# tszalay/poreseq

Hardware: AMD Instinct MI355X
Metric: kb consensus refined/sec at 10x coverage (higher is better)
Workload: dtype f64; 1 GPU; poreseq consensus, 10 kb region, 10x synthetic coverage (BASELINE configs[1]), full Mutate.py schedule per region; a step is 280 independent regions per GPU = 14 lock-step batches; the batches of the timed steps run step by step (a step's batches all finish before the next step's start) through 14 batch slots (host threads) per GPU; marshalling + H2D of the events, host greedy steps and D2H inside; region_bases=10000, events=10, regions_per_gpu=280, batches_in_flight=14, step_barrier=True, parallelism=280 regions x 1 GPU(s), 14 host thread(s) per GPU, no data-path collective

## Files before the change

### poreseq_amd/_capi.py

```python
import ctypes as C
import os

import numpy as np

_HERE = os.path.dirname(os.path.abspath(__file__))
HIP_LIB = os.path.join(_HERE, "csrc", "libporeseq_hip.so")

c_dp = C.POINTER(C.c_double)
c_i32p = C.POINTER(C.c_int32)
c_i64p = C.POINTER(C.c_int64)
c_u8p = C.POINTER(C.c_uint8)


class PsParams(C.Structure):
    _fields_ = [("lik_offset", C.c_double), ("scoring_width", C.c_int32),
                ("realign_width", C.c_int32), ("verbose", C.c_int32)]


class PoreseqError(Exception):
    pass


SYMBOLS = {
    "ps_last_error": (C.c_char_p, []),
    "ps_backend_name": (C.c_char_p, []),
    "ps_info": (C.c_int, [C.c_char_p, C.c_int64]),
    "ps_align_create": (C.c_int, [C.POINTER(C.c_void_p), C.c_char_p, C.c_int64, C.c_int32, c_i64p,
                                  c_dp, c_dp, c_dp, c_dp, c_dp, c_dp, C.c_char_p, c_i64p,
                                  C.POINTER(PsParams)]),
    "ps_align_destroy": (None, [C.c_void_p]),
    "ps_align_set_scoring_width": (C.c_int, [C.c_void_p, C.c_int32]),
    "ps_align_new_call": (C.c_int, [C.c_void_p, C.c_int32]),
    "ps_align_n_events": (C.c_int32, [C.c_void_p]),
    "ps_align_n_levels": (C.c_int64, [C.c_void_p, C.c_int32]),
    "ps_align_sequence_length": (C.c_int64, [C.c_void_p]),
    "ps_align_get_sequence": (C.c_int, [C.c_void_p, C.c_char_p, C.c_int64]),
    "ps_align_get_event_refs": (C.c_int, [C.c_void_p, C.c_int32, c_dp, c_dp]),
    "ps_muts_create": (C.c_int, [C.POINTER(C.c_void_p), C.c_int64, c_i32p, c_i64p, C.c_char_p,
                                 c_i64p, C.c_char_p, c_dp]),
    "ps_muts_destroy": (None, [C.c_void_p]),
    "ps_muts_count": (C.c_int64, [C.c_void_p]),
    "ps_muts_orig_bytes": (C.c_int64, [C.c_void_p]),
    "ps_muts_mut_bytes": (C.c_int64, [C.c_void_p]),
    "ps_muts_export": (C.c_int, [C.c_void_p, c_i32p, c_i64p, C.c_char_p, c_i64p, C.c_char_p, c_dp]),
    "ps_seqs_destroy": (None, [C.c_void_p]),
    "ps_seqs_count": (C.c_int64, [C.c_void_p]),
    "ps_seqs_bytes": (C.c_int64, [C.c_void_p]),
    "ps_seqs_export": (C.c_int, [C.c_void_p, c_i64p, C.c_char_p]),
    "ps_score_alignments": (C.c_int, [C.c_void_p, c_dp, c_dp]),
    "ps_find_point_mutations": (C.c_int, [C.c_void_p, C.POINTER(C.c_void_p)]),
    "ps_find_mutations": (C.c_int, [C.c_void_p, C.c_int32, c_i64p, C.c_char_p, C.POINTER(C.c_void_p)]),
    "ps_score_mutations": (C.c_int, [C.c_void_p, C.c_void_p, C.POINTER(C.c_void_p)]),
    "ps_score_mutation_deltas": (C.c_int, [C.c_void_p, C.c_void_p, c_dp]),
    "ps_make_mutations": (C.c_int, [C.c_void_p, C.c_void_p, c_i32p]),
    "ps_viterbi_mutate": (C.c_int, [C.c_void_p, C.c_int32, C.c_double, C.c_double, C.c_double,
                                    C.c_double, C.c_int32, C.POINTER(C.c_void_p)]),
    "ps_srand": (C.c_int, [C.c_uint32]),
    "ps_rand_draw": (C.c_int, [C.c_int64, c_dp]),
    "ps_rng_create": (C.c_int, [C.POINTER(C.c_void_p), C.c_uint32]),
    "ps_rng_destroy": (None, [C.c_void_p]),
    "ps_seqs_create": (C.c_int, [C.POINTER(C.c_void_p), C.c_int64, c_i64p, C.c_char_p]),
    "ps_batch_score_alignments": (C.c_int, [C.c_int32, C.POINTER(C.c_void_p), C.POINTER(c_dp), C.POINTER(c_dp)]),
    "ps_batch_find_mutations": (C.c_int, [C.c_int32, C.POINTER(C.c_void_p), C.POINTER(C.c_void_p), C.POINTER(C.c_void_p)]),
    "ps_batch_score_mutations": (C.c_int, [C.c_int32, C.POINTER(C.c_void_p), C.POINTER(C.c_void_p), C.POINTER(C.c_void_p)]),
    "ps_batch_make_mutations": (C.c_int, [C.c_int32, C.POINTER(C.c_void_p), C.POINTER(C.c_void_p), c_i32p]),
    "ps_batch_viterbi_mutate": (C.c_int, [C.c_int32, C.POINTER(C.c_void_p), C.POINTER(C.c_void_p), C.c_int32, C.c_double,
                                          C.c_double, C.c_double, C.c_double, C.POINTER(C.c_void_p)]),
    "ps_swfull": (C.c_int, [C.c_char_p, C.c_int64, C.c_char_p, C.c_int64, c_i32p, c_dp, c_i32p,
                            c_i32p, C.c_int64, c_i64p]),
    "ps_seq_to_states": (C.c_int, [C.c_char_p, C.c_int64, c_i32p, c_i64p]),
    "ps_debug_fill": (C.c_int, [C.c_void_p, C.c_int32, C.c_int32, c_dp, c_dp, c_u8p, c_u8p]),
    "ps_set_sweep_min": (C.c_int, [C.c_int32]),
    "ps_set_sweep2_min": (C.c_int, [C.c_int32]),
    "ps_set_sparse_min": (C.c_int, [C.c_int32]),
    "ps_set_sweep_form": (C.c_int, [C.c_int32, C.c_int32]),
    "ps_set_device_fraction": (C.c_int, [C.c_double]),
    "ps_prof_enable": (C.c_int, [C.c_int32]),
    "ps_prof_reset": (C.c_int, []),
    "ps_prof_get": (C.c_int, [C.c_char_p, c_dp, c_i64p, c_dp]),
    "ps_prof_units": (C.c_int, [C.c_char_p, c_dp]),
}


def _dp(a):
    return a.ctypes.data_as(c_dp)


def _f64(a):
    return np.ascontiguousarray(a, dtype=np.float64)


class CApi:

    def __init__(self, path):
        if not os.path.exists(path):
            raise PoreseqError("poreseq_amd: native library not found: %s "
                               "(build it with `python -c 'import __graft_entry__ as g; g.build()'`)" % path)
        self.path = path
        self.lib = C.CDLL(path)
        for name, (res, args) in SYMBOLS.items():
            fn = getattr(self.lib, name)
            fn.restype = res
            fn.argtypes = args

    def check(self, rc):
        if rc != 0:
            msg = self.lib.ps_last_error()
            raise PoreseqError("%s failed (%d): %s" % (os.path.basename(self.path), rc,
                                                      msg.decode() if msg else "?"))

    def backend_name(self):
        return self.lib.ps_backend_name().decode()

    def info(self):
        buf = C.create_string_buffer(1024)
        self.check(self.lib.ps_info(buf, 1024))
        return buf.value.decode()

    def align_create(self, sequence, events, params):
        E = len(events)
        for ev in events:
            ev.makecontiguous()
        lens = [int(ev.mean.size) for ev in events]
        off = np.zeros(E + 1, dtype=np.int64)
        off[1:] = np.cumsum(lens)
        cat = lambda name: (_f64(np.concatenate([_f64(getattr(ev, name)) for ev in events]))
                            if E else np.zeros(0))
        mean, stdv, ra, rl = cat("mean"), cat("stdv"), cat("ref_align"), cat("ref_like")
        for ev, n in zip(events, lens):
            if not (ev.stdv.size == n and ev.ref_align.size == n and ev.ref_like.size == n):
                raise PoreseqError("event arrays differ in length")
        model = np.zeros((E, 4, 1024), dtype=np.float64)
        trans = np.zeros((E, 4), dtype=np.float64)
        for e, ev in enumerate(events):
            m = ev.model
            model[e, 0], model[e, 1] = _f64(m.level_mean), _f64(m.level_stdv)
            model[e, 2], model[e, 3] = _f64(m.sd_mean), _f64(m.sd_stdv)
            trans[e] = (m.prob_skip, m.prob_stay, m.prob_extend, m.prob_insert)
        evseqs = [(getattr(ev, "sequence", "") or "").encode("ascii") for ev in events]
        eoff = np.zeros(E + 1, dtype=np.int64)
        eoff[1:] = np.cumsum([len(s) for s in evseqs])
        epool = b"".join(evseqs)
        pp = PsParams(4.5, 150, 300, 0)
        if "verbose" in params:
            pp.verbose = int(params["verbose"])
        if "lik_offset" in params:
            pp.lik_offset = float(params["lik_offset"])
        if "realign_width" in params:
            pp.realign_width = int(params["realign_width"])
        if "scoring_width" in params:
            pp.scoring_width = int(params["scoring_width"])
        seq = sequence.encode("ascii")
        h = C.c_void_p()
        self.check(self.lib.ps_align_create(C.byref(h), seq, len(seq), E, off.ctypes.data_as(c_i64p),
                                            _dp(mean), _dp(stdv), _dp(ra), _dp(rl), _dp(model),
                                            _dp(trans), epool, eoff.ctypes.data_as(c_i64p), C.byref(pp)))
        return h

    def align_destroy(self, h):
        self.lib.ps_align_destroy(h)

    def align_sequence(self, h):
        n = self.lib.ps_align_sequence_length(h)
        buf = C.create_string_buffer(max(int(n), 1))
        self.check(self.lib.ps_align_get_sequence(h, buf, n))
        return buf.raw[:n].decode("ascii")

    def align_update_events(self, h, events):
        for e, ev in enumerate(events):
            n = int(self.lib.ps_align_n_levels(h, e))
            ra = np.empty(n, dtype=np.float64)
            rl = np.empty(n, dtype=np.float64)
            self.check(self.lib.ps_align_get_event_refs(h, e, _dp(ra), _dp(rl)))
            ev.ref_align[:] = ra
            ev.ref_like[:] = rl

    def muts_create(self, muts, with_scores=False):
        n = len(muts)
        start = np.array([int(m.start) for m in muts], dtype=np.int32)
        origs = [m.orig.encode("ascii") for m in muts]
        mutsb = [m.mut.encode("ascii") for m in muts]
        oo = np.zeros(n + 1, dtype=np.int64)
        oo[1:] = np.cumsum([len(s) for s in origs])
        mo = np.zeros(n + 1, dtype=np.int64)
        mo[1:] = np.cumsum([len(s) for s in mutsb])
        score = np.array([float(m.score) for m in muts], dtype=np.float64) if with_scores else None
        h = C.c_void_p()
        self.check(self.lib.ps_muts_create(C.byref(h), n, start.ctypes.data_as(c_i32p),
                                           oo.ctypes.data_as(c_i64p), b"".join(origs),
                                           mo.ctypes.data_as(c_i64p), b"".join(mutsb),
                                           _dp(score) if score is not None else None))
        return h

    def muts_export(self, h):
        n = int(self.lib.ps_muts_count(h))
        ob, mb = int(self.lib.ps_muts_orig_bytes(h)), int(self.lib.ps_muts_mut_bytes(h))
        start = np.zeros(n, dtype=np.int32)
        oo = np.zeros(n + 1, dtype=np.int64)
        mo = np.zeros(n + 1, dtype=np.int64)
        score = np.zeros(n, dtype=np.float64)
        op = C.create_string_buffer(max(ob, 1))
        mp = C.create_string_buffer(max(mb, 1))
        self.check(self.lib.ps_muts_export(h, start.ctypes.data_as(c_i32p), oo.ctypes.data_as(c_i64p), op,
                                           mo.ctypes.data_as(c_i64p), mp, _dp(score)))
        ops, mps = op.raw[:ob].decode("ascii"), mp.raw[:mb].decode("ascii")
        orig = [ops[oo[i]:oo[i + 1]] for i in range(n)]
        mut = [mps[mo[i]:mo[i + 1]] for i in range(n)]
        return start, orig, mut, score

    def muts_destroy(self, h):
        self.lib.ps_muts_destroy(h)

    def seqs_export(self, h):
        n = int(self.lib.ps_seqs_count(h))
        nb = int(self.lib.ps_seqs_bytes(h))
        off = np.zeros(n + 1, dtype=np.int64)
        pool = C.create_string_buffer(max(nb, 1))
        self.check(self.lib.ps_seqs_export(h, off.ctypes.data_as(c_i64p), pool))
        s = pool.raw[:nb].decode("ascii")
        return [s[off[i]:off[i + 1]] for i in range(n)]

    def score_alignments(self, h, n_events, likes_len=None):
        scores = np.zeros(n_events, dtype=np.float64)
        likes = np.zeros(likes_len, dtype=np.float64) if likes_len is not None else None
        self.check(self.lib.ps_score_alignments(h, _dp(scores), _dp(likes) if likes is not None else None))
        return (scores, likes) if likes is not None else scores

    def find_point_mutations(self, h):
        out = C.c_void_p()
        self.check(self.lib.ps_find_point_mutations(h, C.byref(out)))
        return out

    def find_mutations(self, h, seqs):
        bs = [s.encode("ascii") for s in seqs]
        off = np.zeros(len(bs) + 1, dtype=np.int64)
        off[1:] = np.cumsum([len(b) for b in bs])
        out = C.c_void_p()
        self.check(self.lib.ps_find_mutations(h, len(bs), off.ctypes.data_as(c_i64p), b"".join(bs), C.byref(out)))
        return out

    def score_mutations(self, h, hm):
        out = C.c_void_p()
        self.check(self.lib.ps_score_mutations(h, hm, C.byref(out)))
        return out

    def score_mutation_deltas(self, h, hm, n_events, n_muts):
        out = np.zeros((int(n_events), int(n_muts)), dtype=np.float64)
        if out.size:
            self.check(self.lib.ps_score_mutation_deltas(h, hm, _dp(out)))
        return out

    def make_mutations(self, h, hm):
        nb = C.c_int32(0)
        self.check(self.lib.ps_make_mutations(h, hm, C.byref(nb)))
        return int(nb.value)

    def viterbi_mutate(self, h, nkeep, skip, stay, mmin, mmax, verbose):
        out = C.c_void_p()
        self.check(self.lib.ps_viterbi_mutate(h, nkeep, skip, stay, mmin, mmax, int(bool(verbose)), C.byref(out)))
        try:
            return self.seqs_export(out)
        finally:
            self.lib.ps_seqs_destroy(out)

    @staticmethod
    def _harr(handles):
        arr = (C.c_void_p * len(handles))()
        for i, h in enumerate(handles):
            arr[i] = h.value if isinstance(h, C.c_void_p) else h
        return arr

    def rng_create(self, seed=1):
        h = C.c_void_p()
        self.check(self.lib.ps_rng_create(C.byref(h), int(seed)))
        return h

    def rng_destroy(self, h):
        self.lib.ps_rng_destroy(h)

    def seqs_create(self, seqs):
        bs = [s.encode("ascii") for s in seqs]
        off = np.zeros(len(bs) + 1, dtype=np.int64)
        off[1:] = np.cumsum([len(b) for b in bs])
        h = C.c_void_p()
        self.check(self.lib.ps_seqs_create(C.byref(h), len(bs), off.ctypes.data_as(c_i64p), b"".join(bs)))
        return h

    def seqs_destroy(self, h):
        self.lib.ps_seqs_destroy(h)

    def batch_score_alignments(self, handles, n_events):
        n = len(handles)
        scores = [np.zeros(max(int(e), 1), dtype=np.float64) for e in n_events]
        sp = (c_dp * n)(*[_dp(a) for a in scores])
        self.check(self.lib.ps_batch_score_alignments(n, self._harr(handles), sp, None))
        return [a[:int(e)] for a, e in zip(scores, n_events)]

    def batch_find_mutations(self, handles, seqs_handles):
        n = len(handles)
        out = (C.c_void_p * n)()
        self.check(self.lib.ps_batch_find_mutations(n, self._harr(handles), self._harr(seqs_handles), out))
        return [C.c_void_p(out[i]) for i in range(n)]

    def batch_score_mutations(self, handles, muts_handles):
        n = len(handles)
        out = (C.c_void_p * n)()
        self.check(self.lib.ps_batch_score_mutations(n, self._harr(handles), self._harr(muts_handles), out))
        return [C.c_void_p(out[i]) for i in range(n)]

    def batch_make_mutations(self, handles, muts_handles):
        n = len(handles)
        nb = np.zeros(max(n, 1), dtype=np.int32)
        self.check(self.lib.ps_batch_make_mutations(n, self._harr(handles), self._harr(muts_handles), nb.ctypes.data_as(c_i32p)))
        return [int(x) for x in nb[:n]]

    def batch_viterbi_mutate(self, handles, rngs, nkeep, skip, stay, mmin, mmax):
        n = len(handles)
        out = (C.c_void_p * n)()
        self.check(self.lib.ps_batch_viterbi_mutate(n, self._harr(handles), self._harr(rngs), nkeep, skip, stay, mmin, mmax, out))
        res = []
        for i in range(n):
            h = C.c_void_p(out[i])
            try:
                res.append(self.seqs_export(h))
            finally:
                self.lib.ps_seqs_destroy(h)
        return res

    def srand(self, seed):
        self.check(self.lib.ps_srand(int(seed)))

    def rand_draw(self, n):
        out = np.zeros(int(n), dtype=np.float64)
        self.check(self.lib.ps_rand_draw(int(n), _dp(out)))
        return out

    def swfull(self, s1, s2):
        b1, b2 = s1.encode("ascii"), s2.encode("ascii")
        cap = len(b1) + len(b2) + 1
        i1 = np.zeros(cap, dtype=np.int32)
        i2 = np.zeros(cap, dtype=np.int32)
        score = C.c_int32(0)
        acc = C.c_double(0)
        n = C.c_int64(0)
        self.check(self.lib.ps_swfull(b1, len(b1), b2, len(b2), C.byref(score), C.byref(acc),
                                      i1.ctypes.data_as(c_i32p), i2.ctypes.data_as(c_i32p), cap, C.byref(n)))
        return int(score.value), float(acc.value), i1[:n.value].copy(), i2[:n.value].copy()

    def seq_to_states(self, s):
        b = s.encode("ascii")
        st = np.zeros(max(len(b), 1), dtype=np.int32)
        n = C.c_int64(0)
        self.check(self.lib.ps_seq_to_states(b, len(b), st.ctypes.data_as(c_i32p), C.byref(n)))
        return st[:n.value].copy()

    def debug_fill(self, h, ev, direction, n_levels, n_states):
        shape = (n_levels + 1, n_states + 1)
        main = np.zeros(shape)
        stay = np.zeros(shape)
        sm = np.zeros(shape, dtype=np.uint8)
        ss = np.zeros(shape, dtype=np.uint8)
        self.check(self.lib.ps_debug_fill(h, ev, direction, _dp(main), _dp(stay),
                                          sm.ctypes.data_as(c_u8p), ss.ctypes.data_as(c_u8p)))
        return main, stay, sm, ss

    def set_sweep_min(self, n):
        self.check(self.lib.ps_set_sweep_min(int(n)))

    def set_sweep2_min(self, n):
        self.check(self.lib.ps_set_sweep2_min(int(n)))

    def set_sparse_min(self, n):
        self.check(self.lib.ps_set_sparse_min(int(n)))

    def set_sweep_form(self, rows_per_lane, wavefronts=1):
        self.check(self.lib.ps_set_sweep_form(int(rows_per_lane), int(wavefronts)))

    def set_device_fraction(self, fraction):
        self.check(self.lib.ps_set_device_fraction(float(fraction)))

    def prof_enable(self, on):
        self.check(self.lib.ps_prof_enable(int(on)))

    def prof_reset(self):
        self.check(self.lib.ps_prof_reset())

    def prof_units(self, name):
        u = C.c_double(0)
        self.check(self.lib.ps_prof_units(name.encode(), C.byref(u)))
        return float(u.value)

    def prof_get(self, name):
        ms, n, b = C.c_double(0), C.c_int64(0), C.c_double(0)
        self.check(self.lib.ps_prof_get(name.encode(), C.byref(ms), C.byref(n), C.byref(b)))
        return float(ms.value), int(n.value), float(b.value)


_hip = None


def load_hip():
    global _hip
    if _hip is None:
        _hip = CApi(HIP_LIB)
    return _hip
```

### poreseq_amd/csrc/ps_api.cpp

```cpp
#include <algorithm>
#include <cmath>
#include <cstring>
#include <memory>

#include "ps_host.h"

using namespace ps;

struct ps_align { Align a; };
struct ps_muts { std::vector<Mut> v; };
struct ps_seqs { std::vector<std::string> v; };
struct ps_rng { RandState* s = nullptr; ~ps_rng() { if (s) rand_state_free(s); } };

#define NEED_RT()            \
    Runtime* rt = nullptr;   \
    PS_TRY(runtime(&rt))

extern "C" {

const char* ps_last_error(void) { return last_error(); }
const char* ps_backend_name(void) { return "hip-gfx950"; }
int ps_info(char* out, int64_t cap) {
    if (!out || cap <= 0) return fail(PS_ERR_BAD_ARG, "ps_info");
    const std::string s = info_string();
    const size_t n = std::min<size_t>(s.size(), (size_t)cap - 1);
    memcpy(out, s.data(), n);
    out[n] = 0;
    return PS_OK;
}

int ps_align_create(ps_align** out, const char* seq, int64_t seq_len, int32_t n_events,
                    const int64_t* level_off, const double* mean, const double* stdv,
                    const double* ref_align, const double* ref_like, const double* model,
                    const double* trans, const char* evseq, const int64_t* evseq_off,
                    const ps_params* params) {
    if (!out || !seq || seq_len < 0 || n_events < 0 ||
        (n_events && (!level_off || !mean || !stdv || !ref_align || !ref_like || !model || !trans)))
        return fail(PS_ERR_BAD_ARG, "ps_align_create: bad argument");
    NEED_RT();
    std::unique_ptr<ps_align> h(new ps_align());
    PS_TRY(h->a.create(rt, seq, seq_len, n_events, level_off, mean, stdv, ref_align, ref_like, model, trans,
                       evseq, evseq_off, params));
    *out = h.release();
    return PS_OK;
}
void ps_align_destroy(ps_align* a) { delete a; }
int ps_align_set_scoring_width(ps_align* a, int32_t w) {
    if (!a) return fail(PS_ERR_BAD_ARG, "null handle");
    a->a.par.scoring_width = w;
    return PS_OK;
}
int ps_align_new_call(ps_align* a, int32_t w) {
    if (!a) return fail(PS_ERR_BAD_ARG, "null handle");
    a->a.par.scoring_width = w;
    a->a.seqlikes.clear();
    return PS_OK;
}
int32_t ps_align_n_events(const ps_align* a) { return a ? a->a.E : 0; }
int64_t ps_align_n_levels(const ps_align* a, int32_t e) { return (a && e >= 0 && e < a->a.E) ? a->a.n[e] : -1; }
int64_t ps_align_sequence_length(const ps_align* a) { return a ? (int64_t)a->a.bases.size() : -1; }
int ps_align_get_sequence(const ps_align* a, char* out, int64_t cap) {
    if (!a || !out || cap < (int64_t)a->a.bases.size()) return fail(PS_ERR_BAD_ARG, "ps_align_get_sequence");
    memcpy(out, a->a.bases.data(), a->a.bases.size());
    return PS_OK;
}
int ps_align_get_event_refs(const ps_align* ca, int32_t e, double* ra, double* rl) {
    ps_align* a = const_cast<ps_align*>(ca);
    if (!a || e < 0 || e >= a->a.E) return fail(PS_ERR_BAD_ARG, "ps_align_get_event_refs");
    NEED_RT();
    PS_TRY(a->a.refs_to_host(rt));
    const int64_t o = a->a.off[e];
    if (ra) memcpy(ra, a->a.h_ra.data() + o, a->a.n[e] * sizeof(double));
    if (rl) memcpy(rl, a->a.h_rl.data() + o, a->a.n[e] * sizeof(double));
    return PS_OK;
}

int ps_muts_create(ps_muts** out, int64_t n, const int32_t* start, const int64_t* oo, const char* op,
                   const int64_t* mo, const char* mp, const double* score) {
    if (!out || n < 0 || (n && (!start || !oo || !mo))) return fail(PS_ERR_BAD_ARG, "ps_muts_create");
    ps_muts* m = new ps_muts();
    m->v.resize(n);
    for (int64_t i = 0; i < n; i++) {
        m->v[i].start = start[i];
        if (oo[i + 1] > oo[i]) m->v[i].orig.assign(op + oo[i], op + oo[i + 1]);
        if (mo[i + 1] > mo[i]) m->v[i].mut.assign(mp + mo[i], mp + mo[i + 1]);
        m->v[i].score = score ? score[i] : -1e-6;
    }
    *out = m;
    return PS_OK;
}
void ps_muts_destroy(ps_muts* m) { delete m; }
int64_t ps_muts_count(const ps_muts* m) { return m ? (int64_t)m->v.size() : 0; }
int64_t ps_muts_orig_bytes(const ps_muts* m) { int64_t t = 0; if (m) for (auto& x : m->v) t += x.orig.size(); return t; }
int64_t ps_muts_mut_bytes(const ps_muts* m) { int64_t t = 0; if (m) for (auto& x : m->v) t += x.mut.size(); return t; }
int ps_muts_export(const ps_muts* m, int32_t* start, int64_t* oo, char* op, int64_t* mo, char* mp, double* score) {
    if (!m) return fail(PS_ERR_BAD_ARG, "ps_muts_export");
    int64_t a = 0, b = 0;
    for (size_t i = 0; i < m->v.size(); i++) {
        const Mut& x = m->v[i];
        if (start) start[i] = x.start;
        if (oo) oo[i] = a;
        if (mo) mo[i] = b;
        if (op) memcpy(op + a, x.orig.data(), x.orig.size());
        if (mp) memcpy(mp + b, x.mut.data(), x.mut.size());
        a += x.orig.size(); b += x.mut.size();
        if (score) score[i] = x.score;
    }
    if (oo) oo[m->v.size()] = a;
    if (mo) mo[m->v.size()] = b;
    return PS_OK;
}

void ps_seqs_destroy(ps_seqs* s) { delete s; }
int64_t ps_seqs_count(const ps_seqs* s) { return s ? (int64_t)s->v.size() : 0; }
int64_t ps_seqs_bytes(const ps_seqs* s) { int64_t t = 0; if (s) for (auto& x : s->v) t += x.size(); return t; }
int ps_seqs_export(const ps_seqs* s, int64_t* off, char* pool) {
    if (!s) return fail(PS_ERR_BAD_ARG, "ps_seqs_export");
    int64_t a = 0;
    for (size_t i = 0; i < s->v.size(); i++) {
        if (off) off[i] = a;
        if (pool) memcpy(pool + a, s->v[i].data(), s->v[i].size());
        a += s->v[i].size();
    }
    if (off) off[s->v.size()] = a;
    return PS_OK;
}

int ps_score_alignments(ps_align* a, double* scores, double* likes) {
    if (!a || (!scores && a->a.E)) return fail(PS_ERR_BAD_ARG, "ps_score_alignments");
    NEED_RT();
    return score_alignments(rt, &a->a, scores, likes);
}
int ps_find_point_mutations(ps_align* a, ps_muts** out) {
    if (!a || !out) return fail(PS_ERR_BAD_ARG, "ps_find_point_mutations");
    ps_muts* m = new ps_muts();
    find_point_mutations(&a->a, &m->v);
    *out = m;
    return PS_OK;
}
int ps_find_mutations(ps_align* a, int32_t n, const int64_t* off, const char* pool, ps_muts** out) {
    if (!a || !out || n < 0 || (n && (!off || !pool))) return fail(PS_ERR_BAD_ARG, "ps_find_mutations");
    NEED_RT();
    std::vector<std::string> seeds;
    for (int i = 0; i < n; i++) seeds.emplace_back(pool + off[i], pool + off[i + 1]);
    std::unique_ptr<ps_muts> m(new ps_muts());
    PS_TRY(find_mutations(rt, &a->a, seeds, &m->v));
    *out = m.release();
    return PS_OK;
}
int ps_score_mutations(ps_align* a, const ps_muts* in, ps_muts** out) {
    if (!a || !in || !out) return fail(PS_ERR_BAD_ARG, "ps_score_mutations");
    NEED_RT();
    std::unique_ptr<ps_muts> m(new ps_muts());
    PS_TRY(score_mutations(rt, &a->a, in->v, &m->v));
    *out = m.release();
    return PS_OK;
}
int ps_score_mutation_deltas(ps_align* a, const ps_muts* in, double* deltas) {
    if (!a || !in || !deltas) return fail(PS_ERR_BAD_ARG, "ps_score_mutation_deltas");
    NEED_RT();
    std::vector<Mut> scored;
    std::vector<double*> dout(1, deltas);
    return score_mutations_multi(rt, {&a->a}, {&in->v}, {&scored}, &dout);
}
int ps_make_mutations(ps_align* a, const ps_muts* in, int32_t* nb) {
    if (!a || !in || !nb) return fail(PS_ERR_BAD_ARG, "ps_make_mutations");
    NEED_RT();
    int n = 0;
    PS_TRY(make_mutations(rt, &a->a, in->v, &n));
    *nb = n;
    return PS_OK;
}
int ps_viterbi_mutate(ps_align* a, int32_t nkeep, double skip, double stay, double mmin, double mmax,
                      int32_t verbose, ps_seqs** out) {
    if (!a || !out || a->a.E == 0 || nkeep < 0) return fail(PS_ERR_BAD_ARG, "ps_viterbi_mutate");
    NEED_RT();
    std::unique_ptr<ps_seqs> s(new ps_seqs());
    PS_TRY(viterbi_mutate(rt, &a->a, nkeep, skip, stay, mmin, mmax, &s->v, verbose != 0));
    *out = s.release();
    return PS_OK;
}
int ps_rng_create(ps_rng** out, uint32_t seed) {
    if (!out) return fail(PS_ERR_BAD_ARG, "ps_rng_create");
    ps_rng* r = new ps_rng();
    r->s = rand_state_new(seed);
    *out = r;
    return PS_OK;
}
void ps_rng_destroy(ps_rng* r) { delete r; }
int ps_seqs_create(ps_seqs** out, int64_t n, const int64_t* off, const char* pool) {
    if (!out || n < 0 || (n && (!off || !pool))) return fail(PS_ERR_BAD_ARG, "ps_seqs_create");
    ps_seqs* s = new ps_seqs();
    for (int64_t i = 0; i < n; i++) s->v.emplace_back(pool + off[i], pool + off[i + 1]);
    *out = s;
    return PS_OK;
}
static int batch_handles(int32_t n, ps_align* const* a, std::vector<Align*>* as) {
    if (n < 0 || (n && !a)) return fail(PS_ERR_BAD_ARG, "batch: bad handle array");
    for (int i = 0; i < n; i++) {
        if (!a[i]) return fail(PS_ERR_BAD_ARG, "batch: null handle");
        for (int j = 0; j < i; j++) if (a[j] == a[i]) return fail(PS_ERR_BAD_ARG, "batch: the same handle twice");
        as->push_back(&a[i]->a);
    }
    return PS_OK;
}
int ps_batch_score_alignments(int32_t n, ps_align* const* a, double* const* scores, double* const* likes) {
    std::vector<Align*> as;
    PS_TRY(batch_handles(n, a, &as));
    if (n && !scores) return fail(PS_ERR_BAD_ARG, "ps_batch_score_alignments");
    NEED_RT();
    std::vector<double*> sc(n), lk(n);
    for (int i = 0; i < n; i++) {
        if (!scores[i] && as[i]->E) return fail(PS_ERR_BAD_ARG, "ps_batch_score_alignments: null scores");
        sc[i] = scores[i]; lk[i] = likes ? likes[i] : nullptr;
    }
    return score_alignments_multi(rt, as, sc, lk);
}
int ps_batch_find_mutations(int32_t n, ps_align* const* a, const ps_seqs* const* seeds, ps_muts** out) {
    std::vector<Align*> as;
    PS_TRY(batch_handles(n, a, &as));
    if (n && (!seeds || !out)) return fail(PS_ERR_BAD_ARG, "ps_batch_find_mutations");
    NEED_RT();
    std::vector<std::unique_ptr<ps_muts>> m(n);
    std::vector<const std::vector<std::string>*> sd(n);
    std::vector<std::vector<Mut>*> o(n);
    for (int i = 0; i < n; i++) {
        if (!seeds[i]) return fail(PS_ERR_BAD_ARG, "ps_batch_find_mutations: null seeds");
        m[i].reset(new ps_muts()); sd[i] = &seeds[i]->v; o[i] = &m[i]->v;
    }
    PS_TRY(find_mutations_multi(rt, as, sd, o));
    for (int i = 0; i < n; i++) out[i] = m[i].release();
    return PS_OK;
}
int ps_batch_score_mutations(int32_t n, ps_align* const* a, const ps_muts* const* muts, ps_muts** out) {
    std::vector<Align*> as;
    PS_TRY(batch_handles(n, a, &as));
    if (n && (!muts || !out)) return fail(PS_ERR_BAD_ARG, "ps_batch_score_mutations");
    NEED_RT();
    std::vector<std::unique_ptr<ps_muts>> m(n);
    std::vector<const std::vector<Mut>*> in(n);
    std::vector<std::vector<Mut>*> o(n);
    for (int i = 0; i < n; i++) {
        if (!muts[i]) return fail(PS_ERR_BAD_ARG, "ps_batch_score_mutations: null list");
        m[i].reset(new ps_muts()); in[i] = &muts[i]->v; o[i] = &m[i]->v;
    }
    PS_TRY(score_mutations_multi(rt, as, in, o));
    for (int i = 0; i < n; i++) out[i] = m[i].release();
    return PS_OK;
}
int ps_batch_make_mutations(int32_t n, ps_align* const* a, const ps_muts* const* scored, int32_t* n_bases) {
    std::vector<Align*> as;
    PS_TRY(batch_handles(n, a, &as));
    if (n && (!scored || !n_bases)) return fail(PS_ERR_BAD_ARG, "ps_batch_make_mutations");
    NEED_RT();
    std::vector<std::vector<Mut>> in(n);
    for (int i = 0; i < n; i++) if (!scored[i]) return fail(PS_ERR_BAD_ARG, "ps_batch_make_mutations: null list");
    par_for(n, [&](int i) { in[i] = scored[i]->v; });
    std::vector<int> nb;
    PS_TRY(make_mutations_multi(rt, as, std::move(in), &nb));
    for (int i = 0; i < n; i++) n_bases[i] = nb[i];
    return PS_OK;
}
int ps_batch_viterbi_mutate(int32_t n, ps_align* const* a, ps_rng* const* rng, int32_t nkeep, double skip, double stay,
                            double mmin, double mmax, ps_seqs** out) {
    std::vector<Align*> as;
    PS_TRY(batch_handles(n, a, &as));
    if (n && !out) return fail(PS_ERR_BAD_ARG, "ps_batch_viterbi_mutate");
    if (nkeep < 0) return fail(PS_ERR_BAD_ARG, "ps_batch_viterbi_mutate: nkeep");
    for (Align* x : as) if (x->E == 0) return fail(PS_ERR_BAD_ARG, "ps_batch_viterbi_mutate: no events");
    NEED_RT();
    std::vector<std::unique_ptr<ps_seqs>> s(n);
    std::vector<RandState*> rs(n, nullptr);
    std::vector<std::vector<std::string>*> o(n);
    for (int i = 0; i < n; i++) { s[i].reset(new ps_seqs()); o[i] = &s[i]->v; rs[i] = (rng && rng[i]) ? rng[i]->s : nullptr; }
    PS_TRY(viterbi_mutate_multi(rt, as, rs, nkeep, skip, stay, mmin, mmax, o));
    for (int i = 0; i < n; i++) out[i] = s[i].release();
    return PS_OK;
}

int ps_swfull(const char* s1, int64_t n1, const char* s2, int64_t n2, int32_t* score, double* acc,
              int32_t* i1, int32_t* i2, int64_t cap, int64_t* np) {
    if (!s1 || !s2 || n1 < 0 || n2 < 0 || !np) return fail(PS_ERR_BAD_ARG, "ps_swfull");
    NEED_RT();
    int sc = 0; double ac = 0;
    std::vector<int> a, b;
    PS_TRY(sw_device(rt, std::string(s1, n1), std::string(s2, n2), &sc, &ac, &a, &b));
    if ((int64_t)a.size() > cap) return fail(PS_ERR_BAD_ARG, "ps_swfull: index capacity too small");
    if (score) *score = sc;
    if (acc) *acc = ac;
    for (size_t k = 0; k < a.size(); k++) { if (i1) i1[k] = a[k]; if (i2) i2[k] = b[k]; }
    *np = (int64_t)a.size();
    return PS_OK;
}
int ps_seq_to_states(const char* seq, int64_t n, int32_t* st, int64_t* ns) {
    if (!seq || n < 0 || !ns) return fail(PS_ERR_BAD_ARG, "ps_seq_to_states");
    std::vector<int> v = states_of(std::string(seq, n));
    if (st) std::copy(v.begin(), v.end(), st);
    *ns = (int64_t)v.size();
    return PS_OK;
}

int ps_debug_fill(ps_align* a, int32_t e, int32_t dir, double* main, double* stay, uint8_t* sm, uint8_t* ss) {
    if (!a || e < 0 || e >= a->a.E || !main || dir < 0 || dir > 1) return fail(PS_ERR_BAD_ARG, "ps_debug_fill");
    NEED_RT();
    return debug_fill(rt, &a->a, e, dir, main, stay, sm, ss);
}

int ps_srand(uint32_t seed) { rand_seed(seed); return PS_OK; }
int ps_rand_draw(int64_t n, double* out) {
    if (n < 0 || (n && !out)) return fail(PS_ERR_BAD_ARG, "ps_rand_draw");
    for (int64_t k = 0; k < n; k++) out[k] = rand_next() / (double(RAND_MAX) + 1);
    return PS_OK;
}

int ps_set_sweep_min(int32_t n) { sweep_min_set(n); return PS_OK; }
int ps_set_sweep2_min(int32_t n) { sweep2_min_set(n); return PS_OK; }
int ps_set_sparse_min(int32_t n) { sparse_min_set(n); return PS_OK; }
int ps_set_device_fraction(double f) {
    if (f > 1.0) return fail(PS_ERR_BAD_ARG, "ps_set_device_fraction: a fraction in (0, 1]; <= 0 restores the default");
    device_fraction_set(f);
    return PS_OK;
}
int ps_set_sweep_form(int32_t K, int32_t NW) {
    if (K <= 0 && NW > 0 && NW != 1 && NW != 2 && NW != 4) return fail(PS_ERR_BAD_ARG, "ps_set_sweep_form: 1, 2 or 4 wavefronts per sweep");
    if (K > 0 && !sweep_form_exists(K, NW)) return fail(PS_ERR_BAD_ARG, "ps_set_sweep_form: no such form (rows per lane, wavefronts)");
    sweep_form_set(K, NW);
    return PS_OK;
}

int ps_prof_enable(int32_t on) {
    NEED_RT();
    prof_flush(rt);
    rt->prof_on = on != 0;
    rt->prof_defer = on == 2;
    return PS_OK;
}
int ps_prof_reset(void) {
    NEED_RT();
    prof_flush(rt);
    rt->prof.clear();
    return PS_OK;
}
int ps_prof_get(const char* name, double* ms, int64_t* n, double* bytes) {
    NEED_RT();
    prof_flush(rt);
    Prof p;
    if (name) { auto it = rt->prof.find(name); if (it != rt->prof.end()) p = it->second; }
    if (ms) *ms = p.ms;
    if (n) *n = p.launches;
    if (bytes) *bytes = p.bytes;
    return PS_OK;
}

int ps_prof_units(const char* name, double* units) {
    NEED_RT();
    prof_flush(rt);
    Prof p;
    if (name) { auto it = rt->prof.find(name); if (it != rt->prof.end()) p = it->second; }
    if (units) *units = p.units;
    return PS_OK;
}

}
```

### poreseq_amd/csrc/ps_find.cpp

```cpp
#include <algorithm>
#include <cmath>
#include <cstdlib>
#include <cstring>
#include <map>
#include <thread>

#include "ps_host.h"
#include "ps_sw.h"

namespace ps {

static double max_batch_bytes() { return device_share_bytes(); }

static void fillinds(SwResult& al) {
    if (al.a.empty()) return;
    int i1 = al.a[0], i2 = al.b[0];
    for (size_t k = 0; k < al.a.size(); k++) {
        if (al.a[k] > 0) i1 = al.a[k]; else al.a[k] = i1;
        if (al.b[k] > 0) i2 = al.b[k]; else al.b[k] = i2;
    }
}

static int argmax(const std::vector<double>& v) { return (int)(std::max_element(v.begin(), v.end()) - v.begin()); }

static int extract_edits(Align* a, const std::vector<std::string>& seeds, std::vector<SwResult>& als, const std::vector<double>& base,
                         std::vector<Mut>* out) {
    const size_t L = a->bases.size();
    const int S = (int)seeds.size();
    std::vector<std::vector<double>> dl(S);
    for (int k = 0; k < S; k++) {
        SwResult& al = als[k];
        const std::vector<double>& rl = a->seqlikes[seeds[k]];
        for (size_t q = 0; q < al.a.size(); q++) { al.a[q] -= 2; al.b[q] -= 2; }
        while (!al.a.empty() && (al.a[0] < 0 || al.b[0] < 0)) { al.a.erase(al.a.begin()); al.b.erase(al.b.begin()); }
        const size_t n = al.a.size();
        std::vector<double> x(n), y(n);
        for (size_t q = 0; q < n; q++) {
            x[q] = (size_t)al.a[q] < base.size() ? base[al.a[q]] : 0.0;
            y[q] = (size_t)al.b[q] < rl.size() ? rl[al.b[q]] : 0.0;
        }
        for (size_t q = n; q-- > 1;) { x[q] -= x[q - 1]; y[q] -= y[q - 1]; }
        if (n) { x[0] = 0; y[0] = 0; }
        std::vector<double>& cs = dl[k];
        cs.resize(n);
        double run = 0;
        for (size_t q = 0; q < n; q++) {
            run += y[q] - x[q];
            if (run < 0) run = 0;
            cs[q] = run;
            if (std::fabs(x[q] - y[q]) < 1e-5) cs[q] = 0;
        }
    }
    const size_t BLK = 128;
    std::vector<std::vector<double>> bmax(S);
    auto block_refresh = [&](int k, size_t blk) {
        const std::vector<double>& v = dl[k];
        const size_t lo = blk * BLK, hi = std::min(v.size(), lo + BLK);
        double m = v[lo];
        for (size_t q = lo + 1; q < hi; q++) if (v[q] > m) m = v[q];
        bmax[k][blk] = m;
    };
    auto seed_argmax = [&](int k) -> int {
        const std::vector<double>& bm = bmax[k];
        size_t bb = 0;
        for (size_t q = 1; q < bm.size(); q++) if (bm[q] > bm[bb]) bb = q;
        const std::vector<double>& v = dl[k];
        const size_t lo = bb * BLK, hi = std::min(v.size(), lo + BLK);
        size_t at = lo;
        for (size_t q = lo + 1; q < hi; q++) if (v[q] > v[at]) at = q;
        return (int)at;
    };
    std::vector<double> top(S, 0.0);
    std::vector<int> topi(S, 0);
    for (int k = 0; k < S; k++) {
        if (dl[k].empty()) continue;
        bmax[k].resize((dl[k].size() + BLK - 1) / BLK);
        for (size_t blk = 0; blk < bmax[k].size(); blk++) block_refresh(k, blk);
        topi[k] = seed_argmax(k);
        top[k] = dl[k][topi[k]];
    }
    while (out->size() < L / 3) {
        const int w = argmax(top);
        std::vector<double>& v = dl[w];
        if (v.empty()) break;
        const int ind = topi[w];
        if (v[ind] < 0.25) break;
        int i1 = (int)(std::find(v.begin() + ind, v.end(), 0.0) - v.begin());
        int i0 = -1;
        for (int q = ind; q >= 0; q--) if (v[q] == 0) { i0 = q; break; }
        if (i0 < 0) i0 = 0;
        if (i1 < 0) i1 = 0;
        if ((size_t)i0 >= v.size()) i0 = (int)v.size() - 1;
        if ((size_t)i1 >= v.size()) i1 = (int)v.size() - 1;
        const int s1 = als[w].a[i0], s2 = als[w].b[i0], e1 = als[w].a[ind], e2 = als[w].b[ind];
        Mut m;
        m.start = s1;
        if ((size_t)s1 > a->bases.size() || (size_t)s2 > seeds[w].size()) return PS_ERR_BAD_ARG;
        m.orig = a->bases.substr(s1, (size_t)(e1 - s1));
        m.mut = seeds[w].substr(s2, (size_t)(e2 - s2));
        while (!m.orig.empty() && !m.mut.empty() && m.orig.front() == m.mut.front()) {
            m.orig.erase(m.orig.begin()); m.mut.erase(m.mut.begin()); m.start++;
        }
        while (!m.orig.empty() && !m.mut.empty() && m.orig.back() == m.mut.back()) { m.orig.pop_back(); m.mut.pop_back(); }
        if (!m.orig.empty() || !m.mut.empty()) out->push_back(m);
        std::fill(v.begin() + i0, v.begin() + i1 + 1, 0.0);
        for (size_t blk = (size_t)i0 / BLK; blk <= (size_t)i1 / BLK; blk++) block_refresh(w, blk);
        topi[w] = seed_argmax(w);
        top[w] = v[topi[w]];
    }
    return PS_OK;
}

int find_mutations_multi(Runtime* rt, const std::vector<Align*>& as, const std::vector<const std::vector<std::string>*>& seeds,
                         const std::vector<std::vector<Mut>*>& outs) {
    Tick tk("find_mutations");
    const int R = (int)as.size();
    for (int r = 0; r < R; r++) outs[r]->clear();
    std::vector<std::pair<const std::string*, const std::string*>> pairs;
    std::vector<int> pair0(R + 1, 0);
    for (int r = 0; r < R; r++) {
        pair0[r] = (int)pairs.size();
        for (const std::string& s : *seeds[r]) pairs.push_back({&as[r]->bases, &s});
    }
    pair0[R] = (int)pairs.size();
    auto sw_bytes = [&](size_t k) {
        const double n1 = (double)pairs[k].first->size(), n2 = (double)pairs[k].second->size();
        return 4.0 * ((n1 / 64 + 1) * (n2 + 8) + (n2 / 64 + 1) * (n1 + 1)) + 8.0 * (n1 + n2 + 2);
    };
    double sw_cap = device_share_bytes() / 8;
    auto sw_chunk_end = [&](size_t k0) {
        double acc = 0;
        size_t k = k0;
        for (; k < pairs.size(); k++) { const double add = sw_bytes(k); if (k > k0 && acc + add > sw_cap) break; acc += add; }
        return k;
    };
    typedef std::vector<std::pair<const std::string*, const std::string*>> SwIn;
    SwJob swjob;
    size_t sw_first = sw_chunk_end(0);
    {
        const int rc = sw_launch(rt, SwIn(pairs.begin(), pairs.begin() + sw_first), &swjob);
        if (rc == PS_ERR_NOMEM && sw_first > 1) { sw_first = 0; swjob = SwJob(); }
        else PS_TRY(rc);
    }
    tk.lap("sw enqueue");
    std::vector<std::vector<double>> base(R), sc(R);
    std::vector<double*> scp(R), lkp(R);
    for (int r = 0; r < R; r++) {
        base[r].assign(std::max<size_t>(as[r]->bases.size(), 4) + 1, 0.0);
        sc[r].assign(std::max(as[r]->E, 1), 0.0);
        scp[r] = sc[r].data(); lkp[r] = base[r].data();
    }
    const int rc_base = score_alignments_multi(rt, as, scp, lkp);
    tk.lap("base realign");
    std::vector<SwResult> als_all;
    PS_TRY(sw_finish(rt, &swjob, &als_all));
    PS_TRY(rc_base);
    for (size_t k0 = sw_first; k0 < pairs.size();) {
        const size_t k1 = sw_chunk_end(k0);
        std::vector<SwResult> part;
        const int rc = sw_batch(rt, SwIn(pairs.begin() + k0, pairs.begin() + k1), &part);
        if (rc == PS_ERR_NOMEM && k1 - k0 > 1) { sw_cap *= 0.5; continue; }
        PS_TRY(rc);
        for (SwResult& r : part) als_all.push_back(std::move(r));
        k0 = k1;
    }
    if (sw_first < pairs.size()) { static const bool trace = getenv("PORESEQ_TRACE") != nullptr; if (trace) fprintf(stderr, "[ps] smith-waterman: %zu pairs, %zu with the realign, the rest in chunks\n", pairs.size(), sw_first); }
    if (pairs.empty()) return PS_OK;
    if (R == 1 && as[0]->par.verbose) {
        fputs("Finding mutations", stderr);
        for (size_t k = 0; k < seeds[0]->size(); k++) fputc('.', stderr);
        fputc('\n', stderr);
        fflush(stderr);
    }
    par_for((int)als_all.size(), [&](int k) { fillinds(als_all[k]); });
    tk.lap("smith-waterman");
    struct Need { int r, k; std::vector<int> states; };
    std::vector<Need> need;
    for (int r = 0; r < R; r++) {
        Align* a = as[r];
        const std::vector<std::string>& sd = *seeds[r];
        std::map<std::string, int> seen;
        for (int k = 0; k < (int)sd.size(); k++) {
            if (!a->seqlikes[sd[k]].empty()) continue;
            if (seen.count(sd[k])) continue;
            seen[sd[k]] = k;
            if (a->E) need.push_back({r, k, {}});
            else a->seqlikes[sd[k]] = std::vector<double>(sd[k].size(), 0.0);
        }
    }
    if (!need.empty()) {
        {
            for (int r = 0; r < R; r++) PS_TRY(as[r]->refs_to_host_async(rt));
            PS_HIP(hipStreamSynchronize(rt->stream));
            for (int r = 0; r < R; r++) as[r]->refs_finish();
        }
        par_for((int)need.size(), [&](int q) { need[q].states = states_of((*seeds[need[q].r])[need[q].k]); });
        const double cap = max_batch_bytes();
        size_t q0 = 0;
        int p_seen = 0;
        size_t limit = (size_t)-1;
        while (q0 < need.size()) {
            size_t q1 = q0;
            double bytes = 0;
            size_t nref = 0;
            while (q1 < need.size()) {
                const Align* a = as[need[q1].r];
                const int P = std::max(p_seen, guess_slots(a));
                double add = 0;
                for (int e = 0; e < a->E; e++)
                    add += sweep_enabled() && sweep_guess_k(a->par.realign_width) ? fwd_job_bytes(a, a->n[e], (int)need[q1].states.size())
                                                                                  : ((double)a->n[e] + need[q1].states.size() + 1 + MAT_FRONT + MAT_BACK) * P * 18.0;
                if (q1 > q0 && (bytes + add > cap || q1 - q0 >= limit)) break;
                bytes += add; nref += (size_t)a->ntot; q1++;
            }
            const size_t stage_mark = rt->stage.mark();
            double* h_ra = (double*)rt->stage.alloc(std::max<size_t>(nref, 1) * sizeof(double));
            if (!h_ra) return fail(PS_ERR_NOMEM, "hipHostMalloc (staging arena)");
            std::vector<size_t> roff(q1 - q0 + 1, 0);
            for (size_t q = q0; q < q1; q++) roff[q - q0 + 1] = roff[q - q0] + (size_t)as[need[q].r]->ntot;
            par_for((int)(q1 - q0), [&](int qq) {
                const Need& nd = need[q0 + qq];
                const Align* a = as[nd.r];
                const SwResult& al = als_all[pair0[nd.r] + nd.k];
                double* dst = h_ra + roff[qq];
                for (int64_t t = 0; t < a->ntot; t++) {
                    const int ra = (int)a->h_ra[t];
                    double v = 0.0;
                    if (!al.a.empty() && !(ra < al.a.front() || ra > al.a.back())) {
                        const size_t k = std::lower_bound(al.a.begin(), al.a.end(), ra) - al.a.begin();
                        v = k < al.b.size() ? (double)al.b[k] : 0.0;
                    }
                    dst[t] = v;
                }
            });
            tk.lap("remap (host)");
            DBuf& rb = rt->buf("seed_refs");
            PS_TRY(rb.ensure((size_t)3 * std::max<size_t>(nref, 1) * sizeof(double)));
            double* d_ra = rb.as<double>();
            double* d_rl = d_ra + nref;
            double* d_ri = d_rl + nref;
            if (nref) PS_HIP(hipMemcpyAsync(d_ra, h_ra, nref * sizeof(double), hipMemcpyHostToDevice, rt->stream));
            PS_HIP(hipMemsetAsync(d_rl, 0, std::max<size_t>(nref, 1) * sizeof(double), rt->stream));
            size_t njobs = 0;
            for (size_t q = q0; q < q1; q++) njobs += as[need[q].r]->E;
            DBuf& ob = rt->buf("seed_out");
            PS_TRY(ob.ensure(njobs * sizeof(JobOut)));
            PS_HIP(hipMemsetAsync(ob.p, 0, njobs * sizeof(JobOut), rt->stream));
            std::vector<JobSpec> specs;
            for (size_t q = q0; q < q1; q++) {
                Align* a = as[need[q].r];
                for (int e = 0; e < a->E; e++) {
                    JobSpec s;
                    s.a = a; s.ev = e; s.states = &need[q].states;
                    const size_t o = roff[q - q0] + a->off[e];
                    s.ra = d_ra + o; s.rl = d_rl + o; s.ri = d_ri + o;
                    s.out = ob.as<JobOut>() + specs.size();
                    specs.push_back(s);
                }
            }
            Batch b;
            PS_TRY(b.build(rt, specs, 1, 0));
            PS_TRY(launch_updaterefs(rt, b.d));
            tk.lap("seed batch build");
            {
                const int rc = realign(rt, b, q1 - q0 > 1 ? 1.2 * cap : 0.0);
                if (rc == PS_SPLIT) {
                    { static const bool trace = getenv("PORESEQ_TRACE") != nullptr; if (trace) fprintf(stderr, "[ps] seed chunk of %zu cut again: %d slots per anti-diagonal, %d guessed\n", q1 - q0, b.P, std::max(p_seen, 0)); }
                    p_seen = std::max(p_seen, b.P);
                    limit = std::max<size_t>(1, (q1 - q0) / 2);
                    PS_HIP(hipStreamSynchronize(rt->stream));
                    rt->stage.release(stage_mark);
                    continue;
                }
                PS_TRY(rc);
            }
            p_seen = std::max(p_seen, b.P);
            std::vector<std::vector<double>> lks(q1 - q0);
            bool on_device = true;
            for (size_t q = q0; q < q1; q++) if ((int)need[q].states.size() > likes_max_states()) on_device = false;
            if (on_device) {
                std::vector<LikeGroup> groups(q1 - q0);
                int64_t out_tot = 0;
                int job = 0;
                for (size_t q = q0; q < q1; q++) {
                    LikeGroup& g = groups[q - q0];
                    const std::string& sd = (*seeds[need[q].r])[need[q].k];
                    g.job0 = job; g.njobs = as[need[q].r]->E; job += g.njobs;
                    g.C = (int)need[q].states.size(); g.len = (int)sd.size();
                    g.out_off = out_tot; out_tot += g.len;
                }
                DBuf& gb = rt->buf("like_groups");
                DBuf& lb = rt->buf("like_out");
                PS_TRY(gb.ensure(groups.size() * sizeof(LikeGroup)));
                PS_TRY(lb.ensure((size_t)std::max<int64_t>(out_tot, 1) * sizeof(double)));
                PS_TRY(rt->up(gb.p, groups.data(), groups.size() * sizeof(LikeGroup)));
                PS_TRY(launch_likes(rt, b.d, gb.as<LikeGroup>(), (int)groups.size(), lb.as<double>()));
                double* h_lk = nullptr;
                PS_TRY(rt->down(&h_lk, lb.p, (size_t)out_tot));
                PS_HIP(hipStreamSynchronize(rt->stream));
                tk.lap("seed realign + D2H");
                for (size_t q = q0; q < q1; q++) lks[q - q0].assign(h_lk + groups[q - q0].out_off, h_lk + groups[q - q0].out_off + groups[q - q0].len);
            } else {
            double *r_ra = nullptr, *r_rl = nullptr;
            PS_TRY(rt->down(&r_ra, d_ra, nref));
            PS_TRY(rt->down(&r_rl, d_rl, nref));
            PS_HIP(hipStreamSynchronize(rt->stream));
            tk.lap("seed realign + D2H");
            par_for((int)(q1 - q0), [&](int qq) {
                const Need& nd = need[q0 + qq];
                const Align* a = as[nd.r];
                const std::string& sd = (*seeds[nd.r])[nd.k];
                std::vector<double>& lk = lks[qq];
                lk.assign(std::max<size_t>(sd.size(), 4) + 1, 0.0);
                for (int e = 0; e < a->E; e++) {
                    const size_t o = roff[qq] + a->off[e];
                    accumulate_likes(r_ra + o, r_rl + o, a->n[e], (int)nd.states.size(), lk.data());
                }
                lk.resize(sd.size());
            });
            }
            for (size_t q = q0; q < q1; q++) as[need[q].r]->seqlikes[(*seeds[need[q].r])[need[q].k]] = std::move(lks[q - q0]);
            rt->stage.release(stage_mark);
            q0 = q1;
        }
    }
    tk.lap("seed likes");
    std::vector<int> rcs(R, PS_OK);
    par_for(R, [&](int r) {
        std::vector<SwResult> als(als_all.begin() + pair0[r], als_all.begin() + pair0[r + 1]);
        rcs[r] = extract_edits(as[r], *seeds[r], als, base[r], outs[r]);
    });
    for (int r = 0; r < R; r++) if (rcs[r] != PS_OK) return fail(rcs[r], "FindMutations: alignment index outside the sequence");
    tk.lap("extract");
    return PS_OK;
}

int find_mutations(Runtime* rt, Align* a, const std::vector<std::string>& seeds, std::vector<Mut>* out) {
    return find_mutations_multi(rt, {a}, {&seeds}, {out});
}

inline int succ(int st, int k, int j) { return ((st << (2 * j)) & (NS - 1)) + k; }
inline char base_at(int st, int k) { return "ACGT"[3 & (st >> (2 * (4 - k)))]; }

static std::string path_to_bases(const std::vector<int>& st) {
    std::string s;
    int cur = st[0];
    s.push_back(base_at(cur, 0));
    for (size_t i = 1; i < st.size(); i++) {
        if (cur == st[i]) continue;
        bool hit = false;
        for (int n = 1; n <= 4 && !hit; n++)
            for (int k = 0; k < (1 << (2 * n)); k++)
                if (succ(cur, k, n) == st[i]) {
                    for (int b = 1; b <= n; b++) s.push_back(base_at(cur, b));
                    cur = st[i]; hit = true; break;
                }
        if (!hit) { cur = st[i]; s.push_back(base_at(cur, 0)); }
    }
    for (int b = 1; b <= 4; b++) s.push_back(base_at(cur, b));
    return s;
}

struct RandState {
    random_data rd;
    char st[128];
    bool init = false;
};
namespace { thread_local RandState t_rand; }
static void rs_seed(RandState* r, unsigned seed) {
    memset(&r->rd, 0, sizeof(r->rd));
    initstate_r(seed, r->st, sizeof(r->st), &r->rd);
    r->init = true;
}
static int rs_next(RandState* r) {
    if (!r->init) rs_seed(r, 1);
    int32_t v = 0;
    random_r(&r->rd, &v);
    return (int)v;
}
void rand_seed(unsigned seed) { rs_seed(&t_rand, seed); }
int rand_next() { return rs_next(&t_rand); }
RandState* rand_state_new(unsigned seed) { RandState* r = new RandState(); rs_seed(r, seed); return r; }
void rand_state_free(RandState* r) { delete r; }
void rand_state_seed(RandState* r, unsigned seed) { rs_seed(r, seed); }
int rand_state_next(RandState* r) { return rs_next(r ? r : &t_rand); }

namespace {
struct VitGather { std::vector<double> obsin; int T = 0; };
}

static void vit_gather(const Align* a, const double* h_ri, const JobOut* info, VitGather* g) {
    const int E = a->E;
    int maxpos = 0;
    for (int e = 0; e < E; e++) {
        if (!info[e].has_index) continue;
        const double* ri = h_ri + a->off[e];
        for (int t = 0; t < a->n[e]; t++) {
            const double v = ri[t];
            if (v >= 0.0 && v < 1e9 && v == std::floor(v)) maxpos = std::max(maxpos, (int)v);
        }
    }
    std::vector<std::vector<int>> first(E);
    for (int e = 0; e < E; e++) {
        if (!info[e].has_index) continue;
        first[e].assign((size_t)maxpos + 1, -1);
        const double* ri = h_ri + a->off[e];
        for (int t = 0; t < a->n[e]; t++) {
            const double v = ri[t];
            if (v >= 0.0 && v <= (double)maxpos && v == std::floor(v)) {
                int& slot = first[e][(size_t)v];
                if (slot < 0) slot = t;
            }
        }
    }
    auto rstart = [&](int e) { return info[e].has_index ? info[e].refstart : -1; };
    auto rend = [&](int e) { return info[e].has_index ? info[e].refend : -1; };
    int refind = rstart(0);
    for (int e = 0; e < E; e++) refind = std::min(refind, rstart(e));
    std::vector<double>& obsin = g->obsin;
    int T = 0;
    while (true) {
        int nl = 0, nal = 0;
        const size_t at = obsin.size();
        obsin.resize(at + (size_t)E * 4, 0.0);
        for (int e = 0; e < E; e++) {
            if (refind < 0 || refind > maxpos || first[e].empty() || first[e][refind] < 0) continue;
            const double* ra = a->h_ra.data() + a->off[e];
            const double* mean = a->h_mean.data() + a->off[e];
            const double* stdv = a->h_stdv.data() + a->off[e];
            int t = first[e][refind], cnt = 1;
            double lsum = 0, ssum = 0;
            lsum += mean[t]; ssum += stdv[t];
            for (t++; t < a->n[e] && ra[t] <= refind; t++)
                if (ra[t] > 0) { lsum += mean[t]; ssum += stdv[t]; cnt++; }
            const double lvl = lsum / cnt, sd = ssum / cnt;
            nl++;
            double* o = obsin.data() + at + (size_t)e * 4;
            o[0] = lvl; o[1] = sd; o[2] = std::log(sd); o[3] = 1.0;
        }
        for (int e = 0; e < E; e++) if (refind >= rstart(e) && refind <= rend(e)) nal++;
        if (nl <= nal * 0.2) {
            obsin.resize(at);
            if (nal == 0) break;
            refind++;
            continue;
        }
        T++;
        refind++;
    }
    g->T = T;
}

static void vit_draw(void* rng, double* rnd, size_t n) {
    RandState* r = (RandState*)rng;
    for (size_t k = 0; k < n; k++) rnd[k] = rand_state_next(r) / (double(RAND_MAX) + 1);
}

int viterbi_mutate_multi(Runtime* rt, const std::vector<Align*>& as, const std::vector<RandState*>& rngs, int nkeep, double skip, double stay,
                         double mmin, double mmax, const std::vector<std::vector<std::string>*>& outs) {
    Tick tk("viterbi_mutate");
    const int R = (int)as.size();
    for (int r = 0; r < R; r++) outs[r]->clear();
    std::vector<double*> h_ri(R, nullptr);
    std::vector<JobOut*> info(R, nullptr);
    for (int r = 0; r < R; r++) {
        PS_TRY(as[r]->refs_to_host_async(rt));
        as[r]->last_stream = (void*)rt->stream;
        PS_TRY(rt->down(&h_ri[r], as[r]->d_ri, (size_t)as[r]->ntot));
        PS_TRY(rt->down(&info[r], as[r]->d_out, (size_t)as[r]->E));
    }
    PS_HIP(hipStreamSynchronize(rt->stream));
    for (int r = 0; r < R; r++) as[r]->refs_finish();
    tk.lap("refs D2H");
    std::vector<VitGather> gath(R);
    par_for(R, [&](int r) { vit_gather(as[r], h_ri[r], info[r], &gath[r]); });
    tk.lap("gather levels");
    std::vector<VitRegionH> regs(R);
    for (int r = 0; r < R; r++) {
        regs[r].E = as[r]->E; regs[r].T = gath[r].T; regs[r].obsin = gath[r].obsin.data(); regs[r].d_model = as[r]->d_model;
        as[r]->last_stream = (void*)rt->stream;
        regs[r].rng = rngs[r]; regs[r].draw = vit_draw;
    }
    std::vector<std::vector<std::vector<int>>> paths;
    {
        auto need = [&](size_t k) { return 26.0 * 1024.0 * (double)regs[k].T + 32.0 * (double)regs[k].T * regs[k].E; };
        double cap = std::max(1e9, 0.9 * device_share_bytes());
        for (size_t k0 = 0; k0 < regs.size();) {
            size_t k1 = k0;
            double acc = 0;
            for (; k1 < regs.size(); k1++) { const double add = need(k1); if (k1 > k0 && acc + add > cap) break; acc += add; }
            std::vector<std::vector<std::vector<int>>> part;
            const int rc = viterbi_device_multi(rt, std::vector<VitRegionH>(regs.begin() + k0, regs.begin() + k1), nkeep, skip, stay, mmin, mmax, &part);
            if (rc == PS_ERR_NOMEM && k1 - k0 > 1) { cap *= 0.5; continue; }
            PS_TRY(rc);
            for (auto& pr : part) paths.push_back(std::move(pr));
            k0 = k1;
        }
    }
    tk.lap("device");
    par_for(R, [&](int r) { for (auto& p : paths[r]) outs[r]->push_back(path_to_bases(p)); });
    tk.lap("paths to bases");
    return PS_OK;
}

int viterbi_mutate(Runtime* rt, Align* a, int nkeep, double skip, double stay, double mmin, double mmax,
                   std::vector<std::string>* out, bool verbose) {
    const int rc = viterbi_mutate_multi(rt, {a}, {nullptr}, nkeep, skip, stay, mmin, mmax, {out});
    if (verbose && rc == PS_OK) {
        fputs("Viterbi", stderr);
        for (size_t k = 200; k <= a->bases.size(); k += 200) fputc('.', stderr);
        fputc('\n', stderr);
        fflush(stderr);
    }
    return rc;
}

}
```

### poreseq_amd/csrc/ps_internal.h

```cpp
#ifndef PS_INTERNAL_H_
#define PS_INTERNAL_H_

#include <hip/hip_runtime.h>
#include <stdint.h>

#include <map>
#include <string>
#include <vector>

#include "../../include/poreseq_hip.h"

namespace ps {

constexpr int NS = PS_N_STATES;
constexpr double BIG = 1e300;

int fail(int code, const std::string& msg);
#define PS_HIP(expr)                                                                          \
    do {                                                                                      \
        hipError_t _e = (expr);                                                               \
        if (_e != hipSuccess)                                                                 \
            return ps::fail(PS_ERR_HIP, std::string(#expr) + ": " + hipGetErrorString(_e));   \
    } while (0)
#define PS_TRY(expr)            \
    do {                        \
        int _rc = (expr);       \
        if (_rc != PS_OK) return _rc; \
    } while (0)

struct DBuf {
    void* p = nullptr;
    size_t cap = 0;
    int ensure(size_t bytes);
    template <class T> T* as() const { return (T*)p; }
};

struct HBuf {
    void* p = nullptr;
    size_t cap = 0;
    int ensure(size_t bytes);
    template <class T> T* as() const { return (T*)p; }
};

struct Stage {
    struct Chunk { char* p; size_t cap; };
    std::vector<Chunk> chunks;
    size_t used = 0;
    bool dirty = false;
    void* alloc(size_t bytes);
    int reset();
    size_t mark() const { return chunks.size() <= 1 ? used : (size_t)-1; }
    void release(size_t m) { if (m != (size_t)-1 && chunks.size() <= 1) used = m; }
};

struct Prof { double ms = 0; int64_t launches = 0; double bytes = 0; double units = 0; };

struct Runtime {
    bool ready = false;
    int device = 0;
    hipStream_t stream = nullptr;
    hipStream_t stream2 = nullptr;
    hipEvent_t ev0 = nullptr, ev1 = nullptr, sw0 = nullptr, sw1 = nullptr;
    std::map<std::string, DBuf> pool;
    std::map<std::string, HBuf> hpool;
    HBuf& hbuf(const std::string& name) { return hpool[name]; }
    std::map<std::string, Prof> prof;
    bool prof_on = false;
    bool prof_defer = false;
    struct ProfPend { hipEvent_t a, b; const char* name; double bytes; };
    std::vector<ProfPend> prof_pend;
    std::vector<hipEvent_t> prof_spare;
    DBuf& buf(const std::string& name) { return pool[name]; }
    Stage stage;
    int up(void* dst, const void* src, size_t bytes, hipStream_t st = nullptr);
    int down(void** hptr, const void* src, size_t bytes, hipStream_t st = nullptr);
    template <class T> int down(T** hptr, const void* src, size_t count) { return down((void**)hptr, src, count * sizeof(T)); }
};
int runtime(Runtime** out);
int second_stream(Runtime* rt, hipStream_t* out);
int live_runtimes();

struct Mut {
    int start = 0;
    std::string orig, mut;
    double score = -1e-6;
};

struct JobOut;
struct JobD {
    const double* model8;
    const double* lev[2];
    const int* st;
    double lsk, lst, lex, lin;
    double lik_offset;
    int n0;
    int C;
    int W;
    int force_inert;
    int P;
    int lbn;
    int K;
    int pitch;
    int NL;
    const int* keep[2];
    int64_t lb_off;
    int64_t lbn_off;
    int64_t mat_off[2];
    int64_t lo_off[2];
    int64_t col_off[2];
    int64_t S;
    double* ra;
    double* rl;
    double* ri;
    JobOut* out;
};

struct JobOut {
    double best;
    int bi, bj;
    int has_index;
    int refstart, refend;
    int inert;
    int term_i, term_w;
};

constexpr int MODEL_ROW_BYTES = 80;
constexpr int MAT_FRONT = 8;
constexpr int MAT_BACK = 16;
constexpr int LO_PAD = 160;

struct SweepJob;
struct BatchD {
    const JobD* jobs;
    int njobs;
    int* lb;
    int* lo;
    int* hi;
    double2* rec;
    unsigned short* flg;
    double* cmax;
    double* pm;
    int* maxw;
    int fastdiv;
    double log2pi;
    const SweepJob* s_sj;
    const int2* s_band;
    const int* s_qlo;
    const int* s_qhi;
};

struct StripBest;
struct SweepJob {
    int64_t codes_off;
    int64_t band_off;
    int64_t q_off;
    int64_t sb_off;
    int T;
    int Q;
};
struct SweepD {
    const SweepJob* sj;
    int2* band;
    int* qlo;
    int* qhi;
    unsigned char* codes;
    StripBest* sb;
    int* maxwin;
    int K;
    int nl;
    int ndir;
    int sparse;
};

struct LikeGroup {
    int job0, njobs;
    int C, len;
    int64_t out_off;
};

int launch_updaterefs(Runtime* rt, const BatchD& b);
int launch_lb(Runtime* rt, const BatchD& b, int which , int maxlbn);
int launch_lo(Runtime* rt, const BatchD& b, int ndir, int64_t maxS);
int launch_fill(Runtime* rt, const BatchD& b, const std::vector<JobD>& jobs, int ndir, int64_t maxS, int P, int64_t ncols);
int launch_backtrace(Runtime* rt, const BatchD& b, int maxn);
int launch_prefix(Runtime* rt, const BatchD& b, int ndir);

struct ScoreArgs {
    int job0, njobs;
    int nitems_per_job;
    int ncolmax;
    int ws;
    const int* m_start;
    const int* m_mlen;
    const int* m_cm;
    const int* m_ncol;
    const int* m_skip;
    const int* m_states;
    const int* m_oldidx;
    const int* r0;
    int nr0;
    double* old;
    double* oldall;
    int64_t oldall_pitch, maxS;
    double* delta;
    double* score;
    const int* cls_items[5];
    int cls_count[5];
};
constexpr int SCORE_CLASSES = 5;
int launch_score(Runtime* rt, const BatchD& b, const ScoreArgs* d_sas, const std::vector<ScoreArgs>& h_sas);
int launch_begin(Runtime* rt, const BatchD& b);
int launch_gather_best(Runtime* rt, const BatchD& b, double* out);

int sw_device(Runtime* rt, const std::string& s1, const std::string& s2, int* score, double* accuracy,
              std::vector<int>* inds1, std::vector<int>* inds2);

struct VitRegionH {
    int E = 0, T = 0;
    const double* obsin = nullptr;
    const double* d_model = nullptr;
    void* rng = nullptr;
    void (*draw)(void* rng, double* out , size_t n) = nullptr;
};
int viterbi_device_multi(Runtime* rt, const std::vector<VitRegionH>& regions, int nkeep, double skip, double stay, double mmin, double mmax,
                         std::vector<std::vector<std::vector<int>>>* paths);

void prof_flush(Runtime* rt);
void prof_begin(Runtime* rt);
void prof_end(Runtime* rt, const char* name, double alg_bytes);

}

#endif
```

### poreseq_amd/csrc/ps_sw.h

```cpp
#ifndef PS_SW_H_
#define PS_SW_H_
#include "ps_internal.h"

namespace ps {

struct SwPair {
    int n1, n2;
    int nrb;
    int ngw;
    int pitch;
    int pad;
    int64_t s1_off, s2_off;
    int64_t row_off;
    int64_t col_off;
    int64_t blk_off;
    int64_t out_off;
    int64_t res_off;
};

struct SwResult { int score = 0; double accuracy = 0; std::vector<int> a, b; };

struct SwJob {
    std::vector<SwPair> pairs;
    std::string pool;
    int* res = nullptr;
    int* outbuf = nullptr;
    int64_t out_tot = 0;
    double cells = 0;
    int np = 0;
    hipStream_t stream = nullptr;
};

typedef std::vector<std::pair<const std::string*, const std::string*>> SwInput;
int sw_launch(Runtime* rt, const SwInput& in, SwJob* job);
int sw_finish(Runtime* rt, SwJob* job, std::vector<SwResult>* out);
int sw_batch(Runtime* rt, const SwInput& in, std::vector<SwResult>* out);

}
#endif
```

### poreseq_amd/csrc/ps_sw.hip

```cpp
#include <cstring>

#include "ps_sw.h"

namespace ps {

constexpr int SWB = 8;
constexpr int SWW = 8;
constexpr int SWW1 = 16;

__device__ __forceinline__ int wave_scan_max(int v) {
    asm("s_nop 1\n\tv_max_i32_dpp %0, %0, %0 row_shr:1 row_mask:0xf bank_mask:0xf\n\t"
        "s_nop 1\n\tv_max_i32_dpp %0, %0, %0 row_shr:2 row_mask:0xf bank_mask:0xf\n\t"
        "s_nop 1\n\tv_max_i32_dpp %0, %0, %0 row_shr:4 row_mask:0xf bank_mask:0xf\n\t"
        "s_nop 1\n\tv_max_i32_dpp %0, %0, %0 row_shr:8 row_mask:0xf bank_mask:0xf\n\t"
        "s_nop 1\n\tv_max_i32_dpp %0, %0, %0 row_bcast:15 row_mask:0xa bank_mask:0xf\n\t"
        "s_nop 1\n\tv_max_i32_dpp %0, %0, %0 row_bcast:31 row_mask:0xc bank_mask:0xf"
        : "+v"(v));
    return v;
}

template <int K, int MODE>
__device__ __forceinline__ unsigned sw_row(int (&G)[K], const int (&c2)[K], const int c1, const int bl, const int bprev,
                                           const int lane, const int lane0, const int target, const int i, const int jfirst, int& fc, int& fr) {
    const int d0 = __builtin_amdgcn_update_dpp(bprev + 8 * (K - 1), G[K - 1], 0x138 , 0xf, 0xf, false);
    int y[K];
    int sd0 = 0, up0 = 0;
#pragma unroll
    for (int k = 0; k < K; k++) {
        const int pen = min(c2[k] ^ c1, 9);
        const int sd = (k ? G[k - 1] + 13 : d0 + (5 - 8 * (K - 1))) - pen;
        const int up = G[k] - 8;
        if (k == 0) { sd0 = sd; up0 = up; }
        y[k] = max(max(sd, up), 8 * k);
    }
    constexpr int NG = (K + 3) / 4;
    int tg[NG];
#pragma unroll
    for (int g = 0; g < NG; g++) {
#pragma unroll
        for (int k = 4 * g + 1; k < min(4 * g + 4, K); k++) y[k] = max(y[k], y[k - 1]);
        const int last = y[min(4 * g + 3, K - 1)];
        tg[g] = g ? max(last, tg[g - 1]) : last;
    }
    int z = tg[NG - 1] + (8 * K * lane - 8 * (K - 1));
    z = max(z, (bl - 8 * K) + lane0);
    z = wave_scan_max(z);
    const int hl8 = __builtin_amdgcn_update_dpp(bl - 8 * K, z, 0x138, 0xf, 0xf, false) + (8 * K - 8 * K * lane - 8);
    unsigned code = 0;
#pragma unroll
    for (int k = 0; k < K; k++) {
        const int gn = k >= 4 ? max(max(y[k], tg[k / 4 - 1]), hl8) : max(y[k], hl8);
        if (MODE == 2 && k == 0) {
            const int l0 = max(hl8, 0), m = max(l0, up0);
            const unsigned step = sd0 >= m ? 3u : (up0 > l0 ? 2u : (hl8 > 0 ? 1u : 0u));
            code = step | (gn > 0 ? 4u : 0u) | (c2[0] == c1 ? 8u : 0u);
        }
        if (MODE == 1) {
            const int col = jfirst + k + 1;
            if (gn == target + 8 * k && col < fc) { fc = col; fr = i; }
        }
        G[k] = gn;
    }
    return code;
}

constexpr int SW_SPIN_LIMIT = 1 << 22;
template <int K, int WW>
__global__ __launch_bounds__(64 * WW) void k_sw_fill(const SwPair* pairs, const char* chars, int* rowsave, int* colsave,
                                                  int* blkmax, int* prog, int* ticket, int* res) {
    __shared__ int s_ticket;
    if (threadIdx.x == 0) s_ticket = atomicAdd(&ticket[blockIdx.y], 1);
    __syncthreads();
    const int ss = s_ticket;
    const SwPair p = pairs[blockIdx.y];
    if (p.n1 <= 0 || p.n2 <= 0 || ss * WW * 64 * K >= p.n2) return;
    int* prog_my = prog + (int64_t)blockIdx.y * gridDim.x + ss;
    const bool has_next = (ss + 1) * WW * 64 * K < p.n2;
    int seen = 0;
    const int t = threadIdx.x, w = t >> 6, l = t & 63;
    const int gw = ss * WW + w;
    const int wfirst = gw * 64 * K;
    const bool wave_on = wfirst < p.n2;
    const int jbase = wfirst + l * K;
    const char* s1 = chars + p.s1_off;
    const char* s2 = chars + p.s2_off;
    int c2[K], G[K], bmk[K];
#pragma unroll
    for (int k = 0; k < K; k++) { c2[k] = jbase + k < p.n2 ? (int)(unsigned char)s2[jbase + k] << 4 : 0; G[k] = 8 * k; bmk[k] = 0; }
    const int lane0 = l ? -(1 << 29) : 0;
    __shared__ int hand[WW][2][SWB];
    const bool keeps = ((jbase + K) & 63) == 0 && jbase + K <= p.n2;
    int* csave = colsave + p.col_off + (int64_t)((jbase + K) >> 6) * (p.n1 + 1);
    const int* cprev = colsave + p.col_off + (int64_t)(wfirst >> 6) * (p.n1 + 1);
    if (wave_on && keeps) csave[0] = 0;
    int bprev = 0, dummy_c = 0, dummy_r = 0;
    const int nchunks = (p.n1 + SWB - 1) / SWB;
    auto fetch = [&](int c, int& ch, int& bd) {
        ch = 1; bd = 0;
        const int i0 = c * SWB;
        if (w == 0 && ss > 0 && c >= 0 && c < nchunks) {
            const int need = min(p.n1, (i0 + SWB + 63) & ~63);
            int spins = 0;
            for (; seen < need && spins < SW_SPIN_LIMIT; spins++) {
                seen = __hip_atomic_load(prog_my - 1, __ATOMIC_ACQUIRE, __HIP_MEMORY_SCOPE_AGENT);
                if (seen < need) __builtin_amdgcn_s_sleep(8);
            }
            if (seen < need && l == 0) atomicOr(&res[p.res_off + 5], 1);
        }
        if (wave_on && c >= 0 && c < nchunks && l < SWB && i0 + l < p.n1) {
            ch = (int)(unsigned char)s1[i0 + l] << 4;
            if (w == 0 && gw > 0) bd = cprev[i0 + 1 + l];
        }
    };
    int ch_nx, bd_nx;
    fetch(0 - w, ch_nx, bd_nx);
    for (int s = 0; s < nchunks + WW - 1; s++) {
        const int c = s - w;
        const int ch1 = ch_nx, bd1 = bd_nx;
        fetch(c + 1, ch_nx, bd_nx);
        if (wave_on && c >= 0 && c < nchunks) {
            const int i0 = c * SWB;
            int bnd = bd1;
            if (w > 0 && l < SWB && i0 + l < p.n1) bnd = hand[w - 1][(s - 1) & 1][l];
            int hl[SWB];
#pragma unroll
            for (int r = 0; r < SWB; r++) hl[r] = 0;
#pragma unroll
            for (int r = 0; r < SWB; r++) {
                if (i0 + r < p.n1) {
                    const int bl = __builtin_amdgcn_readlane(bnd, r), c1 = __builtin_amdgcn_readlane(ch1, r);
                    sw_row<K, 0>(G, c2, c1, bl, bprev, l, lane0, 0, 0, 0, dummy_c, dummy_r);
                    bprev = bl;
#pragma unroll
                    for (int k = 0; k < K; k++) bmk[k] = max(bmk[k], G[k]);
                    const int hlast = G[K - 1] - 8 * (K - 1);
                    if (l == 63) hand[w][s & 1][r] = hlast;
                    hl[r] = hlast;
                }
            }
            if (keeps) {
                if (i0 + SWB <= p.n1) {
                    typedef int v4i_a4 __attribute__((ext_vector_type(4), aligned(4)));
                    *(v4i_a4*)(csave + i0 + 1) = (v4i_a4){hl[0], hl[1], hl[2], hl[3]};
                    *(v4i_a4*)(csave + i0 + 5) = (v4i_a4){hl[4], hl[5], hl[6], hl[7]};
                } else {
#pragma unroll
                    for (int r = 0; r < SWB; r++) if (i0 + r < p.n1) csave[i0 + r + 1] = hl[r];
                }
            }
            const int iend = min(i0 + SWB, p.n1);
            if ((iend & 63) == 0 || iend == p.n1) {
                const int q = (iend - 1) >> 6;
                int bm = 0;
#pragma unroll
                for (int k = 0; k < K; k++) { bm = max(bm, bmk[k] - 8 * k); bmk[k] = 0; }
                for (int o = 32; o; o >>= 1) bm = max(bm, __shfl_xor(bm, o));
                if (l == 0) blkmax[p.blk_off + (int64_t)q * p.ngw + gw] = bm;
                if (has_next && w == WW - 1 && l == 63) __hip_atomic_store(prog_my, iend, __ATOMIC_RELEASE, __HIP_MEMORY_SCOPE_AGENT);
                if (iend < p.n1) {
                    int* rs = rowsave + p.row_off + (int64_t)(q + 1) * p.pitch + jbase;
#pragma unroll
                    for (int k = 0; k < K; k++) if (jbase + k < p.n2) rs[k] = G[k] - 8 * k;
                }
            }
        }
        asm volatile("s_waitcnt lgkmcnt(0)\n\ts_barrier" ::: "memory");
    }
}

typedef unsigned short us2 __attribute__((ext_vector_type(2)));
__device__ __forceinline__ us2 pk_of(unsigned v) { return __builtin_bit_cast(us2, v); }
__device__ __forceinline__ unsigned un_pk(us2 v) { return __builtin_bit_cast(unsigned, v); }
constexpr int PKK = 8;
constexpr int SW_PK_MAXLEN = 13000;

__device__ __forceinline__ void sw_row_pk(unsigned (&P)[4], const unsigned (&sp)[4], const int bl, const int bprev, const int lane8k, const int lane0) {
    const int plast = (int)(P[3] >> 16);
    const int d0 = __builtin_amdgcn_update_dpp(bprev + 8 * PKK, plast, 0x138 , 0xf, 0xf, false) - 8 * PKK;
    us2 y[4];
#pragma unroll
    for (int m = 0; m < 4; m++) {
        const unsigned S = m ? __builtin_amdgcn_alignbit(P[m], P[m - 1], 16) : ((P[0] << 16) | (unsigned)d0);
        const us2 sd = pk_of(S) + pk_of(sp[m]);
        const us2 up = __builtin_elementwise_sub_sat(pk_of(P[m]), (us2){8, 8});
        const us2 fl = {(unsigned short)(8 * (2 * m + 1)), (unsigned short)(8 * (2 * m + 2))};
        y[m] = __builtin_elementwise_max(__builtin_elementwise_max(sd, up), fl);
    }
#pragma unroll
    for (int m = 0; m < 4; m++) {
        const us2 lo = {y[m].x, y[m].x};
        y[m] = __builtin_elementwise_max(y[m], lo);
        if (m) { const us2 ph = {y[m - 1].y, y[m - 1].y}; y[m] = __builtin_elementwise_max(y[m], ph); }
    }
    int z = (int)y[3].y + lane8k;
    z = max(z, bl + lane0);
    z = wave_scan_max(z);
    const int hl = __builtin_amdgcn_update_dpp(bl, z, 0x138, 0xf, 0xf, false) - lane8k;
    const us2 hl2 = {(unsigned short)hl, (unsigned short)hl};
#pragma unroll
    for (int m = 0; m < 4; m++) P[m] = un_pk(__builtin_elementwise_max(y[m], hl2));
}

template <int WW>
__global__ __launch_bounds__(64 * WW) __attribute__((amdgpu_waves_per_eu(8, 8))) void k_sw_fill_pk(const SwPair* pairs, const char* chars, int* rowsave, int* colsave,
                                                       int* blkmax, int* prog, int* ticket, int* res) {
    constexpr int K = PKK;
    __shared__ int s_ticket;
    if (threadIdx.x == 0) s_ticket = atomicAdd(&ticket[blockIdx.y], 1);
    __syncthreads();
    const int ss = s_ticket;
    const SwPair p = pairs[blockIdx.y];
    if (p.n1 <= 0 || p.n2 <= 0 || ss * WW * 64 * K >= p.n2) return;
    int* prog_my = prog + (int64_t)blockIdx.y * gridDim.x + ss;
    const bool has_next = (ss + 1) * WW * 64 * K < p.n2;
    int seen = 0;
    const int t = threadIdx.x, w = t >> 6, l = t & 63;
    const int gw = ss * WW + w;
    const int wfirst = gw * 64 * K;
    const bool wave_on = wfirst < p.n2;
    const int jbase = wfirst + l * K;
    const char* s1 = chars + p.s1_off;
    const char* s2 = chars + p.s2_off;
    __shared__ uint4 s_sp[4][64 * WW];
    unsigned P[4], bmk[4], c2p[4];
    {
        unsigned tb[4][4];
#pragma unroll
        for (int m = 0; m < 4; m++) {
            const unsigned a = jbase + 2 * m < p.n2 ? (unsigned)(unsigned char)s2[jbase + 2 * m] : 0u, b = jbase + 2 * m + 1 < p.n2 ? (unsigned)(unsigned char)s2[jbase + 2 * m + 1] : 0u;
            c2p[m] = (a << 4) | (b << 20);
            auto tab = [&](unsigned ch) { return (a == ch ? 13u : 4u) | ((b == ch ? 13u : 4u) << 16); };
            tb[0][m] = tab('A'); tb[1][m] = tab('C'); tb[2][m] = tab('G'); tb[3][m] = tab('T');
            P[m] = (unsigned)(8 * (2 * m + 1)) | ((unsigned)(8 * (2 * m + 2)) << 16);
            bmk[m] = 0u;
        }
#pragma unroll
        for (int q = 0; q < 4; q++) s_sp[q][threadIdx.x] = make_uint4(tb[q][0], tb[q][1], tb[q][2], tb[q][3]);
    }
    const int lane0 = l ? -(1 << 29) : 0, lane8k = 8 * K * l;
    __shared__ int hand[WW][2][SWB];
    const bool keeps = ((jbase + K) & 63) == 0 && jbase + K <= p.n2;
    int* csave = colsave + p.col_off + (int64_t)((jbase + K) >> 6) * (p.n1 + 1);
    const int* cprev = colsave + p.col_off + (int64_t)(wfirst >> 6) * (p.n1 + 1);
    if (wave_on && keeps) csave[0] = 0;
    int bprev = 0;
    const int nchunks = (p.n1 + SWB - 1) / SWB;
    auto fetch = [&](int c, int& ch, int& bd) {
        ch = 1; bd = 0;
        const int i0 = c * SWB;
        if (w == 0 && ss > 0 && c >= 0 && c < nchunks) {
            const int need = min(p.n1, (i0 + SWB + 63) & ~63);
            int spins = 0;
            for (; seen < need && spins < SW_SPIN_LIMIT; spins++) {
                seen = __hip_atomic_load(prog_my - 1, __ATOMIC_ACQUIRE, __HIP_MEMORY_SCOPE_AGENT);
                if (seen < need) __builtin_amdgcn_s_sleep(8);
            }
            if (seen < need && l == 0) atomicOr(&res[p.res_off + 5], 1);
        }
        if (wave_on && c >= 0 && c < nchunks && l < SWB && i0 + l < p.n1) {
            ch = (int)(unsigned char)s1[i0 + l];
            if (w == 0 && gw > 0) bd = cprev[i0 + 1 + l];
        }
    };
    int ch_nx, bd_nx;
    fetch(0 - w, ch_nx, bd_nx);
    for (int s = 0; s < nchunks + WW - 1; s++) {
        const int c = s - w;
        const int ch1 = ch_nx, bd1 = bd_nx;
        fetch(c + 1, ch_nx, bd_nx);
        if (wave_on && c >= 0 && c < nchunks) {
            const int i0 = c * SWB;
            int bnd = bd1;
            if (w > 0 && l < SWB && i0 + l < p.n1) bnd = hand[w - 1][(s - 1) & 1][l];
            int hl[SWB];
#pragma unroll
            for (int r = 0; r < SWB; r++) hl[r] = 0;
#pragma unroll
            for (int r = 0; r < SWB; r++) {
                if (i0 + r < p.n1) {
                    const int bl = __builtin_amdgcn_readlane(bnd, r), c1 = __builtin_amdgcn_readlane(ch1, r);
                    const int bidx = c1 == 'A' ? 0 : c1 == 'C' ? 1 : c1 == 'G' ? 2 : c1 == 'T' ? 3 : -1;
                    unsigned sp[4];
                    if (bidx >= 0) {
                        const uint4 v = s_sp[bidx][threadIdx.x];
                        sp[0] = v.x; sp[1] = v.y; sp[2] = v.z; sp[3] = v.w;
                    } else {
                        const unsigned c1p = ((unsigned)c1 << 4) | ((unsigned)c1 << 20);
#pragma unroll
                        for (int m = 0; m < 4; m++) sp[m] = un_pk((us2){13, 13} - __builtin_elementwise_min(pk_of(c2p[m] ^ c1p), (us2){9, 9}));
                    }
                    sw_row_pk(P, sp, bl, bprev, lane8k, lane0);
                    bprev = bl;
#pragma unroll
                    for (int m = 0; m < 4; m++) bmk[m] = un_pk(__builtin_elementwise_max(pk_of(bmk[m]), pk_of(P[m])));
                    const int hlast = (int)(P[3] >> 16) - 8 * K;
                    if (l == 63) hand[w][s & 1][r] = hlast;
                    hl[r] = hlast;
                }
            }
            if (keeps) {
                if (i0 + SWB <= p.n1) {
                    typedef int v4i_a4 __attribute__((ext_vector_type(4), aligned(4)));
                    *(v4i_a4*)(csave + i0 + 1) = (v4i_a4){hl[0], hl[1], hl[2], hl[3]};
                    *(v4i_a4*)(csave + i0 + 5) = (v4i_a4){hl[4], hl[5], hl[6], hl[7]};
                } else {
#pragma unroll
                    for (int r = 0; r < SWB; r++) if (i0 + r < p.n1) csave[i0 + r + 1] = hl[r];
                }
            }
            const int iend = min(i0 + SWB, p.n1);
            if ((iend & 63) == 0 || iend == p.n1) {
                const int q = (iend - 1) >> 6;
                int bm = 0;
#pragma unroll
                for (int m = 0; m < 4; m++) {
                    bm = max(bm, (int)(bmk[m] & 0xffffu) - 8 * (2 * m + 1));
                    bm = max(bm, (int)(bmk[m] >> 16) - 8 * (2 * m + 2));
                    bmk[m] = 0u;
                }
                for (int o = 32; o; o >>= 1) bm = max(bm, __shfl_xor(bm, o));
                if (l == 0) blkmax[p.blk_off + (int64_t)q * p.ngw + gw] = bm;
                if (has_next && w == WW - 1 && l == 63) __hip_atomic_store(prog_my, iend, __ATOMIC_RELEASE, __HIP_MEMORY_SCOPE_AGENT);
                if (iend < p.n1) {
                    int* rs = rowsave + p.row_off + (int64_t)(q + 1) * p.pitch + jbase;
#pragma unroll
                    for (int m = 0; m < 4; m++) {
                        if (jbase + 2 * m < p.n2) rs[2 * m] = (int)(P[m] & 0xffffu) - 8 * (2 * m + 1);
                        if (jbase + 2 * m + 1 < p.n2) rs[2 * m + 1] = (int)(P[m] >> 16) - 8 * (2 * m + 2);
                    }
                }
            }
        }
        asm volatile("s_waitcnt lgkmcnt(0)\n\ts_barrier" ::: "memory");
    }
}

template <int K, int MODE>
__device__ __forceinline__ void sw_tile(const SwPair& p, const char* s1, const char* s2, const int* rowsave, const int* colsave,
                                        const int q, const int c0, const int nrows, const int l, const int target, int& fc, int& fr,
                                        unsigned char (*codes)[64]) {
    const int jbase = c0 + l * K;
    int c2[K], G[K];
    const int* rs = rowsave + p.row_off + (int64_t)q * p.pitch + jbase;
#pragma unroll
    for (int k = 0; k < K; k++) {
        const bool ok = jbase + k < p.n2;
        c2[k] = ok ? (int)(unsigned char)s2[jbase + k] << 4 : 0;
        G[k] = ((ok && q > 0) ? rs[k] : 0) + 8 * k;
    }
    const int* cprev = colsave + p.col_off + (int64_t)(c0 >> 6) * (p.n1 + 1);
    int bprev = c0 > 0 ? cprev[64 * q] : 0;
    int bnd = 0, ch1 = 1;
    if (l < nrows) { ch1 = (int)(unsigned char)s1[64 * q + l] << 4; if (c0 > 0) bnd = cprev[64 * q + 1 + l]; }
    const int lane0 = l ? -(1 << 29) : 0;
    for (int r = 0; r < nrows; r++) {
        const int bl = __builtin_amdgcn_readlane(bnd, r), c1 = __builtin_amdgcn_readlane(ch1, r);
        const unsigned cd = sw_row<K, MODE>(G, c2, c1, bl, bprev, l, lane0, target, 64 * q + r + 1, jbase, fc, fr);
        if (MODE == 2) codes[r][l] = (unsigned char)cd;
        bprev = bl;
    }
}

template <int K>
__global__ __launch_bounds__(64) __attribute__((amdgpu_waves_per_eu(K <= 8 ? 8 : 4, 8))) void k_sw_trace(const SwPair* pairs, const char* chars, const int* rowsave, const int* colsave,
                                                 const int* blkmax, int* out, int* res) {
    __shared__ unsigned char codes[64][64];
#ifndef PS_WALKER_PRIO
#define PS_WALKER_PRIO 3
#endif
    if (PS_WALKER_PRIO > 0) __builtin_amdgcn_s_setprio(PS_WALKER_PRIO);
    const SwPair p = pairs[blockIdx.x];
    const int l = threadIdx.x;
    int* o = res + p.res_off;
    const char* s1 = chars + p.s1_off;
    const char* s2 = chars + p.s2_off;
    const int* bmx = blkmax + p.blk_off;
    int best = 0;
    if (p.n1 > 0 && p.n2 > 0)
        for (int k = l; k < p.nrb * p.ngw; k += 64) best = max(best, bmx[k]);
    for (int s = 32; s; s >>= 1) best = max(best, __shfl_xor(best, s));
    if (best <= 0) {
        if (l == 0) { o[0] = 0; o[1] = 0; o[2] = 0; o[3] = 0; o[4] = 0; }
        return;
    }
    int bi = 0, bj = 0;
    for (int gw = 0; gw < p.ngw && !bj; gw++) {
        int fc = 0x7fffffff, fr = 0x7fffffff;
        for (int q0 = 0; q0 < p.nrb; q0 += 64) {
            const int q = q0 + l;
            unsigned long long hit = __ballot(q < p.nrb && bmx[(int64_t)q * p.ngw + gw] == best);
            while (hit) {
                const int qq = q0 + (int)__builtin_ctzll(hit);
                hit &= hit - 1;
                sw_tile<K, 1>(p, s1, s2, rowsave, colsave, qq, gw * 64 * K, min(64, p.n1 - 64 * qq), l, best, fc, fr, codes);
            }
        }
        for (int s = 32; s; s >>= 1) {
            const int oc = __shfl_xor(fc, s), orow = __shfl_xor(fr, s);
            if (oc < fc || (oc == fc && orow < fr)) { fc = oc; fr = orow; }
        }
        if (fc != 0x7fffffff) { bj = fc; bi = fr; }
    }
    int* oi = out + p.out_off;
    int* oj = oi + (p.n1 + p.n2 + 2);
    int i = bi, j = bj, np = 0, nm = 0;
    bool done = false;
    while (!done && i > 0 && j > 0) {
        const int q = (i - 1) >> 6, cb = (j - 1) >> 6;
        const int r0 = 64 * q + 1, cfirst = 64 * cb + 1;
        int dc = 0, dr = 0;
        __syncthreads();
        sw_tile<1, 2>(p, s1, s2, rowsave, colsave, q, 64 * cb, i - 64 * q, l, 0, dc, dr, codes);
        __syncthreads();
        while (true) {
            if (!(i > 0 && j > 0)) { done = true; break; }
            if (i < r0 || j < cfirst) break;
            const int ii = i - l, jj = j - l;
            unsigned code = 0;
            if (ii >= r0 && jj >= cfirst) code = codes[ii - r0][jj - cfirst];
            const unsigned long long dm = __ballot((code & 7u) == 7u);
            const int run = __builtin_amdgcn_readfirstlane(dm == ~0ull ? 64 : (int)__builtin_ctzll(~dm));
            if (l < run) { oi[np + l] = ii; oj[np + l] = jj; }
            nm += (int)__popcll(__ballot((code & 8u) && l < run));
            np += run; i -= run; j -= run;
            if (run == 64) continue;
            if (!(i > 0 && j > 0)) { done = true; break; }
            if (i < r0 || j < cfirst) break;
            const unsigned cr = __builtin_amdgcn_readlane(code, run);
            if (!(cr & 4u)) { done = true; break; }
            const unsigned stp = cr & 3u;
            if (stp == 1u) { if (l == 0) { oi[np] = 0; oj[np] = j; } np++; j--; }
            else if (stp == 2u) { if (l == 0) { oi[np] = i; oj[np] = 0; } np++; i--; }
            else { done = true; break; }
        }
    }
    if (l == 0) { o[0] = best; o[1] = bi; o[2] = bj; o[3] = np; o[4] = nm; }
}

static int sw_run_pk(Runtime* rt, hipStream_t st, int np, int nss, const SwPair* d_pairs, const char* d_chars, int* d_row, int* d_col,
                     int* d_blk, int* d_prog, int* d_ticket, int* d_out, int* d_res) {
    static const size_t pad = getenv("PORESEQ_SW_LDS_PAD_KB") ? (size_t)atoi(getenv("PORESEQ_SW_LDS_PAD_KB")) * 1024 : 0;
    hipLaunchKernelGGL((k_sw_fill_pk<SWW>), dim3(nss, np), dim3(64 * SWW), pad, st, d_pairs, d_chars, d_row, d_col, d_blk, d_prog, d_ticket, d_res);
    PS_HIP(hipGetLastError());
    hipLaunchKernelGGL(k_sw_trace<8>, dim3(np), dim3(64), 0, st, d_pairs, d_chars, d_row, d_col, d_blk, d_out, d_res);
    PS_HIP(hipGetLastError());
    return PS_OK;
}

template <int K, int WW>
static int sw_run(Runtime* rt, hipStream_t st, int np, int nss, const SwPair* d_pairs, const char* d_chars, int* d_row, int* d_col,
                  int* d_blk, int* d_prog, int* d_ticket, int* d_out, int* d_res) {
    hipLaunchKernelGGL((k_sw_fill<K, WW>), dim3(nss, np), dim3(64 * WW), 0, st, d_pairs, d_chars, d_row, d_col, d_blk, d_prog, d_ticket, d_res);
    PS_HIP(hipGetLastError());
    hipLaunchKernelGGL(k_sw_trace<K>, dim3(np), dim3(64), 0, st, d_pairs, d_chars, d_row, d_col, d_blk, d_out, d_res);
    PS_HIP(hipGetLastError());
    return PS_OK;
}

int sw_launch(Runtime* rt, const std::vector<std::pair<const std::string*, const std::string*>>& in, SwJob* job) {
    const int np = (int)in.size();
    job->np = np;
    if (!np) return PS_OK;
    std::vector<SwPair>& pairs = job->pairs;
    std::string& pool = job->pool;
    pairs.assign(np, SwPair());
    int maxn2 = 1;
    for (int k = 0; k < np; k++) maxn2 = std::max(maxn2, (int)in[k].second->size());
    int K = live_runtimes() > 1 ? 8 : 4, WW = SWW;
    if (const char* e = getenv("PORESEQ_SW_K")) K = atoi(e) == 16 ? 16 : (atoi(e) == 8 ? 8 : 4);
    {
        const char* form = getenv("PORESEQ_SW_FORM");
        const int k1 = maxn2 <= SWW1 * 64 * 8 ? 8 : (maxn2 <= SWW1 * 64 * 16 ? 16 : 0);
        if (form && !strcmp(form, "one") && k1) { K = k1; WW = SWW1; }
    }
    const int sswidth = WW * 64 * K;
    const int nss = (maxn2 + sswidth - 1) / sswidth;
    int64_t row_tot = 0, col_tot = 0, blk_tot = 0, out_tot = 0;
    for (int k = 0; k < np; k++) {
        SwPair& p = pairs[k];
        p.n1 = (int)in[k].first->size(); p.n2 = (int)in[k].second->size();
        p.nrb = std::max(1, (p.n1 + 63) / 64);
        p.ngw = WW * std::max(1, (p.n2 + sswidth - 1) / sswidth);
        p.pitch = ((p.n2 + 3) / 4) * 4 + 4;
        p.s1_off = (int64_t)pool.size(); pool += *in[k].first;
        p.s2_off = (int64_t)pool.size(); pool += *in[k].second;
        p.row_off = row_tot; row_tot += (int64_t)p.nrb * p.pitch;
        p.col_off = col_tot; col_tot += ((int64_t)p.n2 / 64 + 1) * (p.n1 + 1);
        p.blk_off = blk_tot; blk_tot += (int64_t)p.nrb * p.ngw;
        p.out_off = out_tot; out_tot += 2 * ((int64_t)p.n1 + p.n2 + 2);
        p.res_off = (int64_t)k * 8;
        job->cells += (double)p.n1 * p.n2;
    }
    pool.push_back(0);
    job->out_tot = out_tot;
    PS_TRY(rt->buf("sw_pairs").ensure(np * sizeof(SwPair)));
    PS_TRY(rt->buf("sw_chars").ensure(pool.size()));
    PS_TRY(rt->buf("sw_row").ensure(row_tot * sizeof(int)));
    PS_TRY(rt->buf("sw_col").ensure(col_tot * sizeof(int)));
    PS_TRY(rt->buf("sw_blk").ensure(blk_tot * sizeof(int)));
    PS_TRY(rt->buf("sw_prog").ensure((size_t)np * (nss + 1) * sizeof(int)));
    PS_TRY(rt->buf("sw_out").ensure(out_tot * sizeof(int)));
    PS_TRY(rt->buf("sw_res").ensure((size_t)np * 8 * sizeof(int)));
    SwPair* d_pairs = rt->buf("sw_pairs").as<SwPair>();
    char* d_chars = rt->buf("sw_chars").as<char>();
    int* d_row = rt->buf("sw_row").as<int>();
    int* d_col = rt->buf("sw_col").as<int>();
    int* d_blk = rt->buf("sw_blk").as<int>();
    int* d_prog = rt->buf("sw_prog").as<int>();
    int* d_ticket = d_prog + (size_t)np * nss;
    int* d_out = rt->buf("sw_out").as<int>();
    int* d_res = rt->buf("sw_res").as<int>();
    hipStream_t st = nullptr;
    PS_TRY(second_stream(rt, &st));
    job->stream = st;
    PS_TRY(rt->up(d_pairs, pairs.data(), np * sizeof(SwPair), st));
    PS_TRY(rt->up(d_chars, pool.data(), pool.size(), st));
    PS_HIP(hipMemsetAsync(d_res, 0, (size_t)np * 8 * sizeof(int), st));
    PS_HIP(hipMemsetAsync(d_blk, 0, blk_tot * sizeof(int), st));
    PS_HIP(hipMemsetAsync(d_prog, 0, (size_t)np * (nss + 1) * sizeof(int), st));
    if (rt->prof_on) PS_HIP(hipEventRecord(rt->sw0, st));
    bool packed = K == 8 && WW == SWW;
    for (int k = 0; k < np && packed; k++) if (std::min(pairs[k].n1, pairs[k].n2) > SW_PK_MAXLEN) packed = false;
    if (const char* e = getenv("PORESEQ_SW_PK")) if (atoi(e) == 0) packed = false;
    if (packed) {
        PS_TRY(sw_run_pk(rt, st, np, nss, d_pairs, d_chars, d_row, d_col, d_blk, d_prog, d_ticket, d_out, d_res));
        if (rt->prof_on) rt->prof["sw_pk8"].launches++;
    } else if (WW == SWW1) {
        switch (K) {
            case 8: PS_TRY((sw_run<8, SWW1>(rt, st, np, nss, d_pairs, d_chars, d_row, d_col, d_blk, d_prog, d_ticket, d_out, d_res))); break;
            default: PS_TRY((sw_run<16, SWW1>(rt, st, np, nss, d_pairs, d_chars, d_row, d_col, d_blk, d_prog, d_ticket, d_out, d_res))); break;
        }
    } else {
        switch (K) {
            case 4: PS_TRY((sw_run<4, SWW>(rt, st, np, nss, d_pairs, d_chars, d_row, d_col, d_blk, d_prog, d_ticket, d_out, d_res))); break;
            case 16: PS_TRY((sw_run<16, SWW>(rt, st, np, nss, d_pairs, d_chars, d_row, d_col, d_blk, d_prog, d_ticket, d_out, d_res))); break;
            default: PS_TRY((sw_run<8, SWW>(rt, st, np, nss, d_pairs, d_chars, d_row, d_col, d_blk, d_prog, d_ticket, d_out, d_res))); break;
        }
    }
    if (rt->prof_on) PS_HIP(hipEventRecord(rt->sw1, st));
    PS_TRY(rt->hbuf("sw_res").ensure((size_t)np * 8 * sizeof(int)));
    PS_TRY(rt->hbuf("sw_out").ensure((size_t)out_tot * sizeof(int)));
    job->res = rt->hbuf("sw_res").as<int>();
    job->outbuf = rt->hbuf("sw_out").as<int>();
    PS_HIP(hipMemcpyAsync(job->res, d_res, (size_t)np * 8 * sizeof(int), hipMemcpyDeviceToHost, st));
    PS_HIP(hipMemcpyAsync(job->outbuf, d_out, (size_t)out_tot * sizeof(int), hipMemcpyDeviceToHost, st));
    return PS_OK;
}

int sw_finish(Runtime* rt, SwJob* job, std::vector<SwResult>* out) {
    const int np = job->np;
    out->assign(np, SwResult());
    if (!np) return PS_OK;
    PS_HIP(hipStreamSynchronize(job->stream));
    if (rt->prof_on) {
        float ms = 0;
        if (hipEventElapsedTime(&ms, rt->sw0, rt->sw1) == hipSuccess) {
            Prof& pr = rt->prof["sw"];
            pr.ms += ms; pr.launches += 1; pr.bytes += job->cells * 5.0;
        }
    }
    for (int k = 0; k < np; k++)
        if (job->res[k * 8 + 5]) return fail(PS_ERR_HIP, "Smith-Waterman: a strip gave up waiting for its left neighbour (result discarded)");
    for (int k = 0; k < np; k++) {
        const int n = job->res[k * 8 + 3], nm = job->res[k * 8 + 4];
        const SwPair& p = job->pairs[k];
        SwResult& r = (*out)[k];
        r.score = job->res[k * 8 + 0];
        const int* oi = job->outbuf + p.out_off;
        const int* oj = oi + (p.n1 + p.n2 + 2);
        r.a.assign(oi, oi + n); r.b.assign(oj, oj + n);
        std::reverse(r.a.begin(), r.a.end()); std::reverse(r.b.begin(), r.b.end());
        r.accuracy = 100.0 * nm / (double)n;
    }
    return PS_OK;
}

int sw_batch(Runtime* rt, const std::vector<std::pair<const std::string*, const std::string*>>& in, std::vector<SwResult>* out) {
    SwJob job;
    PS_TRY(sw_launch(rt, in, &job));
    return sw_finish(rt, &job, out);
}

int sw_device(Runtime* rt, const std::string& s1, const std::string& s2, int* score, double* accuracy,
              std::vector<int>* inds1, std::vector<int>* inds2) {
    std::vector<std::pair<const std::string*, const std::string*>> in(1, {&s1, &s2});
    std::vector<SwResult> out;
    PS_TRY(sw_batch(rt, in, &out));
    *score = out[0].score; *accuracy = out[0].accuracy;
    inds1->swap(out[0].a); inds2->swap(out[0].b);
    return PS_OK;
}

}
```

Measured before the change: 203.6 kb/s.

## Add banded Smith-Waterman path with full-matrix fallback for seed alignments

New measurement: 218.7 kb/s (median of 6 runs). 7.4% higher.

```diff
diff --git a/poreseq_amd/_capi.py b/poreseq_amd/_capi.py
--- a/poreseq_amd/_capi.py
+++ b/poreseq_amd/_capi.py
@@ -347,6 +347,13 @@
                                       i1.ctypes.data_as(c_i32p), i2.ctypes.data_as(c_i32p), cap, C.byref(n)))
         return int(score.value), float(acc.value), i1[:n.value].copy(), i2[:n.value].copy()
 
+    def debug_sw_band(self):
+        fn = self.lib.ps_debug_sw_band
+        fn.restype, fn.argtypes = C.c_int, [c_i64p]
+        out = np.zeros(5, dtype=np.int64)
+        self.check(fn(out.ctypes.data_as(c_i64p)))
+        return dict(zip(("banded", "fell_back", "edge", "band_cells", "full_cells"), (int(v) for v in out)))
+
     def seq_to_states(self, s):
         b = s.encode("ascii")
         st = np.zeros(max(len(b), 1), dtype=np.int32)
diff --git a/poreseq_amd/csrc/ps_api.cpp b/poreseq_amd/csrc/ps_api.cpp
--- a/poreseq_amd/csrc/ps_api.cpp
+++ b/poreseq_amd/csrc/ps_api.cpp
@@ -300,6 +300,11 @@
     return PS_OK;
 }
 
+int ps_debug_sw_band(int64_t* out) {
+    if (!out) return fail(PS_ERR_BAD_ARG, "ps_debug_sw_band");
+    sw_band_counters(out);
+    return PS_OK;
+}
 int ps_debug_fill(ps_align* a, int32_t e, int32_t dir, double* main, double* stay, uint8_t* sm, uint8_t* ss) {
     if (!a || e < 0 || e >= a->a.E || !main || dir < 0 || dir > 1) return fail(PS_ERR_BAD_ARG, "ps_debug_fill");
     NEED_RT();
diff --git a/poreseq_amd/csrc/ps_find.cpp b/poreseq_amd/csrc/ps_find.cpp
--- a/poreseq_amd/csrc/ps_find.cpp
+++ b/poreseq_amd/csrc/ps_find.cpp
@@ -123,10 +123,9 @@
         for (const std::string& s : *seeds[r]) pairs.push_back({&as[r]->bases, &s});
     }
     pair0[R] = (int)pairs.size();
-    auto sw_bytes = [&](size_t k) {
-        const double n1 = (double)pairs[k].first->size(), n2 = (double)pairs[k].second->size();
-        return 4.0 * ((n1 / 64 + 1) * (n2 + 8) + (n2 / 64 + 1) * (n1 + 1)) + 8.0 * (n1 + n2 + 2);
-    };
+    std::vector<int> wbs(pairs.size());
+    for (size_t k = 0; k < pairs.size(); k++) wbs[k] = sw_band_choice(*pairs[k].first, *pairs[k].second);
+    auto sw_bytes = [&](size_t k) { return sw_pair_bytes((int)pairs[k].first->size(), (int)pairs[k].second->size(), wbs[k]); };
     double sw_cap = device_share_bytes() / 8;
     auto sw_chunk_end = [&](size_t k0) {
         double acc = 0;
@@ -138,7 +137,7 @@
     SwJob swjob;
     size_t sw_first = sw_chunk_end(0);
     {
-        const int rc = sw_launch(rt, SwIn(pairs.begin(), pairs.begin() + sw_first), &swjob);
+        const int rc = sw_launch(rt, SwIn(pairs.begin(), pairs.begin() + sw_first), &swjob, wbs.data());
         if (rc == PS_ERR_NOMEM && sw_first > 1) { sw_first = 0; swjob = SwJob(); }
         else PS_TRY(rc);
     }
@@ -158,7 +157,7 @@
     for (size_t k0 = sw_first; k0 < pairs.size();) {
         const size_t k1 = sw_chunk_end(k0);
         std::vector<SwResult> part;
-        const int rc = sw_batch(rt, SwIn(pairs.begin() + k0, pairs.begin() + k1), &part);
+        const int rc = sw_batch(rt, SwIn(pairs.begin() + k0, pairs.begin() + k1), &part, wbs.data() + k0);
         if (rc == PS_ERR_NOMEM && k1 - k0 > 1) { sw_cap *= 0.5; continue; }
         PS_TRY(rc);
         for (SwResult& r : part) als_all.push_back(std::move(r));
diff --git a/poreseq_amd/csrc/ps_internal.h b/poreseq_amd/csrc/ps_internal.h
--- a/poreseq_amd/csrc/ps_internal.h
+++ b/poreseq_amd/csrc/ps_internal.h
@@ -214,6 +214,7 @@
 
 int sw_device(Runtime* rt, const std::string& s1, const std::string& s2, int* score, double* accuracy,
               std::vector<int>* inds1, std::vector<int>* inds2);
+void sw_band_counters(int64_t out[5]);
 
 struct VitRegionH {
     int E = 0, T = 0;
diff --git a/poreseq_amd/csrc/ps_sw.h b/poreseq_amd/csrc/ps_sw.h
--- a/poreseq_amd/csrc/ps_sw.h
+++ b/poreseq_amd/csrc/ps_sw.h
@@ -9,7 +9,9 @@
     int nrb;
     int ngw;
     int pitch;
-    int pad;
+    int wb;
+    int nbb;
+    int cpitch;
     int64_t s1_off, s2_off;
     int64_t row_off;
     int64_t col_off;
@@ -27,14 +29,19 @@
     int* outbuf = nullptr;
     int64_t out_tot = 0;
     double cells = 0;
+    double band_cells = 0;
     int np = 0;
+    int nband = 0;
     hipStream_t stream = nullptr;
 };
 
 typedef std::vector<std::pair<const std::string*, const std::string*>> SwInput;
-int sw_launch(Runtime* rt, const SwInput& in, SwJob* job);
+int sw_band_choice(const std::string& s1, const std::string& s2);
+double sw_pair_bytes(int n1, int n2, int wb);
+int sw_launch(Runtime* rt, const SwInput& in, SwJob* job, const int* wb = nullptr);
 int sw_finish(Runtime* rt, SwJob* job, std::vector<SwResult>* out);
-int sw_batch(Runtime* rt, const SwInput& in, std::vector<SwResult>* out);
+int sw_batch(Runtime* rt, const SwInput& in, std::vector<SwResult>* out, const int* wb = nullptr);
+void sw_band_counters(int64_t out[5]);
 
 }
 #endif
diff --git a/poreseq_amd/csrc/ps_sw.hip b/poreseq_amd/csrc/ps_sw.hip
--- a/poreseq_amd/csrc/ps_sw.hip
+++ b/poreseq_amd/csrc/ps_sw.hip
@@ -1,3 +1,4 @@
+#include <atomic>
 #include <cstring>
 
 #include "ps_sw.h"
@@ -7,6 +8,23 @@
 constexpr int SWB = 8;
 constexpr int SWW = 8;
 constexpr int SWW1 = 16;
+constexpr int SWBS = 512;
+constexpr int SWBW = 4;
+
+__device__ __forceinline__ int band_lo(const SwPair& p, int s) { return p.wb ? s * (SWBS / 64) - p.wb / 64 : 0; }
+__device__ __forceinline__ int64_t rs_index(const SwPair& p, int q, int j) {
+    if (!p.wb) return p.row_off + (int64_t)q * p.pitch + j;
+    const int s = j / SWBS;
+    return p.row_off + ((int64_t)s * p.nbb + q - band_lo(p, s)) * SWBS + (j - s * SWBS);
+}
+__device__ __forceinline__ int64_t col_base(const SwPair& p, int c) { return p.col_off + (int64_t)c * p.cpitch - (p.wb ? 64 * band_lo(p, (64 * c - 1) / SWBS) : 0); }
+__device__ __forceinline__ int col_hi(const SwPair& p, int c) { return p.wb ? min(p.n1, 64 * (band_lo(p, (64 * c - 1) / SWBS) + p.nbb)) : p.n1; }
+__device__ __forceinline__ int64_t bm_index(const SwPair& p, int q, int gw) {
+    return p.wb ? p.blk_off + (int64_t)gw * p.nbb + q - band_lo(p, gw) : p.blk_off + (int64_t)q * p.ngw + gw;
+}
+__device__ __forceinline__ int band_q0(const SwPair& p, int gw) { return max(0, band_lo(p, gw)); }
+__device__ __forceinline__ int band_q1(const SwPair& p, int gw) { return p.wb ? min(p.nrb, band_lo(p, gw) + p.nbb) : p.nrb; }
+__device__ __forceinline__ int band_bound(int i, int j, int wb) { return 5 * min(i, j) - 8 * max(0, wb + 1 - abs(i - j)); }
 
 __device__ __forceinline__ int wave_scan_max(int v) {
     asm("s_nop 1\n\tv_max_i32_dpp %0, %0, %0 row_shr:1 row_mask:0xf bank_mask:0xf\n\t"
@@ -54,6 +72,10 @@
             const int l0 = max(hl8, 0), m = max(l0, up0);
             const unsigned step = sd0 >= m ? 3u : (up0 > l0 ? 2u : (hl8 > 0 ? 1u : 0u));
             code = step | (gn > 0 ? 4u : 0u) | (c2[0] == c1 ? 8u : 0u);
+            const int j = jfirst + 1;
+            if (!target || (gn >= band_bound(i, j, target) && hl8 + 8 >= band_bound(i, j - 1, target) &&
+                            up0 + 8 >= band_bound(i - 1, j, target) && d0 >= band_bound(i - 1, j - 1, target)))
+                code |= 16u;
         }
         if (MODE == 1) {
             const int col = jfirst + k + 1;
@@ -201,21 +223,30 @@
     for (int m = 0; m < 4; m++) P[m] = un_pk(__builtin_elementwise_max(y[m], hl2));
 }
 
-template <int WW>
+template <int WW, bool BAND>
 __global__ __launch_bounds__(64 * WW) __attribute__((amdgpu_waves_per_eu(8, 8))) void k_sw_fill_pk(const SwPair* pairs, const char* chars, int* rowsave, int* colsave,
                                                        int* blkmax, int* prog, int* ticket, int* res) {
     constexpr int K = PKK;
-    __shared__ int s_ticket;
-    if (threadIdx.x == 0) s_ticket = atomicAdd(&ticket[blockIdx.y], 1);
+    static_assert(!BAND || 64 * K == SWBS, "band strips are one wave");
+    constexpr int WP = BAND ? 1 : WW;
+    constexpr int KEY = 32768;
+    __shared__ int s_ticket, s_key[WW];
+    if (!BAND) {
+        if (threadIdx.x == 0) s_ticket = atomicAdd(&ticket[blockIdx.y], 1);
+    } else if (threadIdx.x < WW) {
+        s_key[threadIdx.x] = 0;
+    }
     __syncthreads();
-    const int ss = s_ticket;
     const SwPair p = pairs[blockIdx.y];
-    if (p.n1 <= 0 || p.n2 <= 0 || ss * WW * 64 * K >= p.n2) return;
+    const int nstrip = BAND ? (p.n2 + SWBS - 1) / SWBS : 1;
+    for (int it = BAND ? (int)(threadIdx.x >> 6) : 0; it < nstrip; it += BAND ? WW : 1) {
+    const int ss = BAND ? it : s_ticket;
+    if (p.n1 <= 0 || p.n2 <= 0 || ss * WP * 64 * K >= p.n2) return;
     int* prog_my = prog + (int64_t)blockIdx.y * gridDim.x + ss;
-    const bool has_next = (ss + 1) * WW * 64 * K < p.n2;
+    const bool has_next = !BAND && (ss + 1) * WW * 64 * K < p.n2;
     int seen = 0;
-    const int t = threadIdx.x, w = t >> 6, l = t & 63;
-    const int gw = ss * WW + w;
+    const int t = threadIdx.x, w = t >> 6, l = t & 63, wp = BAND ? 0 : w;
+    const int gw = BAND ? ss : ss * WW + w;
     const int wfirst = gw * 64 * K;
     const bool wave_on = wfirst < p.n2;
     const int jbase = wfirst + l * K;
@@ -240,16 +271,28 @@
     const int lane0 = l ? -(1 << 29) : 0, lane8k = 8 * K * l;
     __shared__ int hand[WW][2][SWB];
     const bool keeps = ((jbase + K) & 63) == 0 && jbase + K <= p.n2;
-    int* csave = colsave + p.col_off + (int64_t)((jbase + K) >> 6) * (p.n1 + 1);
-    const int* cprev = colsave + p.col_off + (int64_t)(wfirst >> 6) * (p.n1 + 1);
-    if (wave_on && keeps) csave[0] = 0;
+    const int lo = BAND ? band_lo(p, ss) : 0, q0 = max(0, lo), r0 = 64 * q0;
+    const int rend = BAND ? min(p.n1, 64 * (lo + p.nbb)) : p.n1;
+    const int pend = BAND ? min(p.n1, 64 * (lo - SWBS / 64 + p.nbb)) : p.n1;
+    int* csave = colsave + p.col_off + (int64_t)((jbase + K) >> 6) * p.cpitch - 64 * lo;
+    const int* cprev = colsave + p.col_off + (int64_t)(wfirst >> 6) * p.cpitch - (BAND ? 64 * (lo - SWBS / 64) : 0);
+    if (wave_on && keeps) csave[r0] = 0;
     int bprev = 0;
-    const int nchunks = (p.n1 + SWB - 1) / SWB;
+    const int cb = r0 / SWB, ce = (rend + SWB - 1) / SWB;
     auto fetch = [&](int c, int& ch, int& bd) {
         ch = 1; bd = 0;
         const int i0 = c * SWB;
-        if (w == 0 && ss > 0 && c >= 0 && c < nchunks) {
-            const int need = min(p.n1, (i0 + SWB + 63) & ~63);
+        if (BAND && ss > 0 && c >= cb && c < ce) {
+            const int want = (ss - 1) * KEY + min(pend, (i0 + SWB + 63) & ~63) - 64 * max(0, lo - SWBS / 64);
+            int spins = 0;
+            for (; seen < want && spins < SW_SPIN_LIMIT; spins++) {
+                seen = __hip_atomic_load(&s_key[(w + WW - 1) % WW], __ATOMIC_ACQUIRE, __HIP_MEMORY_SCOPE_WORKGROUP);
+                if (seen < want) __builtin_amdgcn_s_sleep(2);
+            }
+            if (seen < want && l == 0) atomicOr(&res[p.res_off + 5], 1);
+        }
+        if (!BAND && w == 0 && ss > 0 && c >= cb && c < ce) {
+            const int need = min(pend, (i0 + SWB + 63) & ~63);
             int spins = 0;
             for (; seen < need && spins < SW_SPIN_LIMIT; spins++) {
                 seen = __hip_atomic_load(prog_my - 1, __ATOMIC_ACQUIRE, __HIP_MEMORY_SCOPE_AGENT);
@@ -257,27 +300,28 @@
             }
             if (seen < need && l == 0) atomicOr(&res[p.res_off + 5], 1);
         }
-        if (wave_on && c >= 0 && c < nchunks && l < SWB && i0 + l < p.n1) {
+        if (wave_on && c >= cb && c < ce && l < SWB && i0 + l < rend) {
             ch = (int)(unsigned char)s1[i0 + l];
-            if (w == 0 && gw > 0) bd = cprev[i0 + 1 + l];
+            if (wp == 0 && gw > 0 && i0 + 1 + l <= pend) bd = cprev[i0 + 1 + l];
         }
     };
     int ch_nx, bd_nx;
-    fetch(0 - w, ch_nx, bd_nx);
-    for (int s = 0; s < nchunks + WW - 1; s++) {
-        const int c = s - w;
+    fetch(cb - wp, ch_nx, bd_nx);
+    if (BAND && gw > 0 && r0 > 0 && r0 <= pend) bprev = cprev[r0];
+    for (int s = 0; s < ce - cb + WP - 1; s++) {
+        const int c = cb + s - wp;
         const int ch1 = ch_nx, bd1 = bd_nx;
         fetch(c + 1, ch_nx, bd_nx);
-        if (wave_on && c >= 0 && c < nchunks) {
+        if (wave_on && c >= cb && c < ce) {
             const int i0 = c * SWB;
             int bnd = bd1;
-            if (w > 0 && l < SWB && i0 + l < p.n1) bnd = hand[w - 1][(s - 1) & 1][l];
+            if (wp > 0 && l < SWB && i0 + l < rend) bnd = hand[w - 1][(s - 1) & 1][l];
             int hl[SWB];
 #pragma unroll
             for (int r = 0; r < SWB; r++) hl[r] = 0;
 #pragma unroll
             for (int r = 0; r < SWB; r++) {
-                if (i0 + r < p.n1) {
+                if (i0 + r < rend) {
                     const int bl = __builtin_amdgcn_readlane(bnd, r), c1 = __builtin_amdgcn_readlane(ch1, r);
                     const int bidx = c1 == 'A' ? 0 : c1 == 'C' ? 1 : c1 == 'G' ? 2 : c1 == 'T' ? 3 : -1;
                     unsigned sp[4];
@@ -294,22 +338,22 @@
 #pragma unroll
                     for (int m = 0; m < 4; m++) bmk[m] = un_pk(__builtin_elementwise_max(pk_of(bmk[m]), pk_of(P[m])));
                     const int hlast = (int)(P[3] >> 16) - 8 * K;
-                    if (l == 63) hand[w][s & 1][r] = hlast;
+                    if (!BAND && l == 63) hand[w][s & 1][r] = hlast;
                     hl[r] = hlast;
                 }
             }
             if (keeps) {
-                if (i0 + SWB <= p.n1) {
+                if (i0 + SWB <= rend) {
                     typedef int v4i_a4 __attribute__((ext_vector_type(4), aligned(4)));
                     *(v4i_a4*)(csave + i0 + 1) = (v4i_a4){hl[0], hl[1], hl[2], hl[3]};
                     *(v4i_a4*)(csave + i0 + 5) = (v4i_a4){hl[4], hl[5], hl[6], hl[7]};
                 } else {
 #pragma unroll
-                    for (int r = 0; r < SWB; r++) if (i0 + r < p.n1) csave[i0 + r + 1] = hl[r];
+                    for (int r = 0; r < SWB; r++) if (i0 + r < rend) csave[i0 + r + 1] = hl[r];
                 }
             }
-            const int iend = min(i0 + SWB, p.n1);
-            if ((iend & 63) == 0 || iend == p.n1) {
+            const int iend = min(i0 + SWB, rend);
+            if ((iend & 63) == 0 || iend == rend) {
                 const int q = (iend - 1) >> 6;
                 int bm = 0;
 #pragma unroll
@@ -319,10 +363,12 @@
                     bmk[m] = 0u;
                 }
                 for (int o = 32; o; o >>= 1) bm = max(bm, __shfl_xor(bm, o));
-                if (l == 0) blkmax[p.blk_off + (int64_t)q * p.ngw + gw] = bm;
+                if (l == 0) blkmax[BAND ? p.blk_off + (int64_t)gw * p.nbb + q - lo : p.blk_off + (int64_t)q * p.ngw + gw] = bm;
                 if (has_next && w == WW - 1 && l == 63) __hip_atomic_store(prog_my, iend, __ATOMIC_RELEASE, __HIP_MEMORY_SCOPE_AGENT);
-                if (iend < p.n1) {
-                    int* rs = rowsave + p.row_off + (int64_t)(q + 1) * p.pitch + jbase;
+                if (BAND && l == 63) __hip_atomic_store(&s_key[w], ss * KEY + iend - r0, __ATOMIC_RELEASE, __HIP_MEMORY_SCOPE_WORKGROUP);
+                if (iend < rend) {
+                    int* rs = rowsave + (BAND ? p.row_off + ((int64_t)ss * p.nbb + q + 1 - lo) * SWBS + (jbase - ss * SWBS)
+                                              : p.row_off + (int64_t)(q + 1) * p.pitch + jbase);
 #pragma unroll
                     for (int m = 0; m < 4; m++) {
                         if (jbase + 2 * m < p.n2) rs[2 * m] = (int)(P[m] & 0xffffu) - 8 * (2 * m + 1);
@@ -331,7 +377,9 @@
                 }
             }
         }
-        asm volatile("s_waitcnt lgkmcnt(0)\n\ts_barrier" ::: "memory");
+        if (!BAND) asm volatile("s_waitcnt lgkmcnt(0)\n\ts_barrier" ::: "memory");
+    }
+    if (BAND && l == 63) __hip_atomic_store(&s_key[w], (ss + 1) * KEY, __ATOMIC_RELEASE, __HIP_MEMORY_SCOPE_WORKGROUP);
     }
 }
 
@@ -341,17 +389,19 @@
                                         unsigned char (*codes)[64]) {
     const int jbase = c0 + l * K;
     int c2[K], G[K];
-    const int* rs = rowsave + p.row_off + (int64_t)q * p.pitch + jbase;
+    const int* rs = rowsave + rs_index(p, q, jbase);
+    const bool top = q > band_q0(p, c0 / SWBS);
 #pragma unroll
     for (int k = 0; k < K; k++) {
         const bool ok = jbase + k < p.n2;
         c2[k] = ok ? (int)(unsigned char)s2[jbase + k] << 4 : 0;
-        G[k] = ((ok && q > 0) ? rs[k] : 0) + 8 * k;
-    }
-    const int* cprev = colsave + p.col_off + (int64_t)(c0 >> 6) * (p.n1 + 1);
-    int bprev = c0 > 0 ? cprev[64 * q] : 0;
+        G[k] = ((ok && top) ? rs[k] : 0) + 8 * k;
+    }
+    const int* cprev = colsave + col_base(p, c0 >> 6);
+    const int chi = c0 > 0 ? col_hi(p, c0 >> 6) : 0;
+    int bprev = c0 > 0 && 64 * q <= chi ? cprev[64 * q] : 0;
     int bnd = 0, ch1 = 1;
-    if (l < nrows) { ch1 = (int)(unsigned char)s1[64 * q + l] << 4; if (c0 > 0) bnd = cprev[64 * q + 1 + l]; }
+    if (l < nrows) { ch1 = (int)(unsigned char)s1[64 * q + l] << 4; if (c0 > 0 && 64 * q + 1 + l <= chi) bnd = cprev[64 * q + 1 + l]; }
     const int lane0 = l ? -(1 << 29) : 0;
     for (int r = 0; r < nrows; r++) {
         const int bl = __builtin_amdgcn_readlane(bnd, r), c1 = __builtin_amdgcn_readlane(ch1, r);
@@ -377,8 +427,15 @@
     const int* bmx = blkmax + p.blk_off;
     int best = 0;
     if (p.n1 > 0 && p.n2 > 0)
-        for (int k = l; k < p.nrb * p.ngw; k += 64) best = max(best, bmx[k]);
+        for (int k = l; k < (p.wb ? p.nbb : p.nrb) * p.ngw; k += 64) best = max(best, bmx[k]);
     for (int s = 32; s; s >>= 1) best = max(best, __shfl_xor(best, s));
+    if (p.wb) {
+        const int u = 5 * max(0, max(min(p.n1, p.n2 - p.wb - 1), min(p.n2, p.n1 - p.wb - 1)));
+        if (best <= u) {
+            if (l == 0) o[6] = 1;
+            return;
+        }
+    }
     if (best <= 0) {
         if (l == 0) { o[0] = 0; o[1] = 0; o[2] = 0; o[3] = 0; o[4] = 0; }
         return;
@@ -386,9 +443,10 @@
     int bi = 0, bj = 0;
     for (int gw = 0; gw < p.ngw && !bj; gw++) {
         int fc = 0x7fffffff, fr = 0x7fffffff;
-        for (int q0 = 0; q0 < p.nrb; q0 += 64) {
+        const int qa = band_q0(p, gw), qb = band_q1(p, gw);
+        for (int q0 = qa; q0 < qb; q0 += 64) {
             const int q = q0 + l;
-            unsigned long long hit = __ballot(q < p.nrb && bmx[(int64_t)q * p.ngw + gw] == best);
+            unsigned long long hit = __ballot(q < qb && blkmax[bm_index(p, q, gw)] == best);
             while (hit) {
                 const int qq = q0 + (int)__builtin_ctzll(hit);
                 hit &= hit - 1;
@@ -404,13 +462,13 @@
     int* oi = out + p.out_off;
     int* oj = oi + (p.n1 + p.n2 + 2);
     int i = bi, j = bj, np = 0, nm = 0;
-    bool done = false;
+    bool done = false, inexact = false;
     while (!done && i > 0 && j > 0) {
         const int q = (i - 1) >> 6, cb = (j - 1) >> 6;
         const int r0 = 64 * q + 1, cfirst = 64 * cb + 1;
         int dc = 0, dr = 0;
         __syncthreads();
-        sw_tile<1, 2>(p, s1, s2, rowsave, colsave, q, 64 * cb, i - 64 * q, l, 0, dc, dr, codes);
+        sw_tile<1, 2>(p, s1, s2, rowsave, colsave, q, 64 * cb, i - 64 * q, l, p.wb, dc, dr, codes);
         __syncthreads();
         while (true) {
             if (!(i > 0 && j > 0)) { done = true; break; }
@@ -420,6 +478,7 @@
             if (ii >= r0 && jj >= cfirst) code = codes[ii - r0][jj - cfirst];
             const unsigned long long dm = __ballot((code & 7u) == 7u);
             const int run = __builtin_amdgcn_readfirstlane(dm == ~0ull ? 64 : (int)__builtin_ctzll(~dm));
+            if (__ballot(l < run && !(code & 16u))) { inexact = true; done = true; break; }
             if (l < run) { oi[np + l] = ii; oj[np + l] = jj; }
             nm += (int)__popcll(__ballot((code & 8u) && l < run));
             np += run; i -= run; j -= run;
@@ -427,6 +486,7 @@
             if (!(i > 0 && j > 0)) { done = true; break; }
             if (i < r0 || j < cfirst) break;
             const unsigned cr = __builtin_amdgcn_readlane(code, run);
+            if (!(cr & 16u)) { inexact = true; done = true; break; }
             if (!(cr & 4u)) { done = true; break; }
             const unsigned stp = cr & 3u;
             if (stp == 1u) { if (l == 0) { oi[np] = 0; oj[np] = j; } np++; j--; }
@@ -434,13 +494,22 @@
             else { done = true; break; }
         }
     }
-    if (l == 0) { o[0] = best; o[1] = bi; o[2] = bj; o[3] = np; o[4] = nm; }
+    if (l == 0) { o[0] = best; o[1] = bi; o[2] = bj; o[3] = np; o[4] = nm; o[6] = inexact ? 1 : 0; }
 }
 
 static int sw_run_pk(Runtime* rt, hipStream_t st, int np, int nss, const SwPair* d_pairs, const char* d_chars, int* d_row, int* d_col,
                      int* d_blk, int* d_prog, int* d_ticket, int* d_out, int* d_res) {
     static const size_t pad = getenv("PORESEQ_SW_LDS_PAD_KB") ? (size_t)atoi(getenv("PORESEQ_SW_LDS_PAD_KB")) * 1024 : 0;
-    hipLaunchKernelGGL((k_sw_fill_pk<SWW>), dim3(nss, np), dim3(64 * SWW), pad, st, d_pairs, d_chars, d_row, d_col, d_blk, d_prog, d_ticket, d_res);
+    hipLaunchKernelGGL((k_sw_fill_pk<SWW, false>), dim3(nss, np), dim3(64 * SWW), pad, st, d_pairs, d_chars, d_row, d_col, d_blk, d_prog, d_ticket, d_res);
+    PS_HIP(hipGetLastError());
+    hipLaunchKernelGGL(k_sw_trace<8>, dim3(np), dim3(64), 0, st, d_pairs, d_chars, d_row, d_col, d_blk, d_out, d_res);
+    PS_HIP(hipGetLastError());
+    return PS_OK;
+}
+
+static int sw_run_band(Runtime* rt, hipStream_t st, int np, const SwPair* d_pairs, const char* d_chars, int* d_row, int* d_col,
+                       int* d_blk, int* d_out, int* d_res) {
+    hipLaunchKernelGGL((k_sw_fill_pk<SWBW, true>), dim3(1, np), dim3(64 * SWBW), 0, st, d_pairs, d_chars, d_row, d_col, d_blk, nullptr, nullptr, d_res);
     PS_HIP(hipGetLastError());
     hipLaunchKernelGGL(k_sw_trace<8>, dim3(np), dim3(64), 0, st, d_pairs, d_chars, d_row, d_col, d_blk, d_out, d_res);
     PS_HIP(hipGetLastError());
@@ -457,15 +526,91 @@
     return PS_OK;
 }
 
-int sw_launch(Runtime* rt, const std::vector<std::pair<const std::string*, const std::string*>>& in, SwJob* job) {
+constexpr int SW_BAND_W = 1024;
+
+static int band_width_env() {
+    const char* e = getenv("PORESEQ_SW_BAND_W");
+    const int w = e ? atoi(e) : SW_BAND_W;
+    return w >= 64 ? std::min(w, 8192) / 64 * 64 : SW_BAND_W;
+}
+
+static double band_cells(int n1, int n2, int wb) {
+    const int nbb = SWBS / 64 + 2 * wb / 64, ns = (n2 + SWBS - 1) / SWBS, nrb = (n1 + 63) / 64;
+    double c = 0;
+    for (int s = 0; s < ns; s++) {
+        const int lo = s * (SWBS / 64) - wb / 64, r0 = 64 * std::max(0, lo), r1 = std::min(n1, 64 * std::min(nrb, lo + nbb));
+        c += (double)std::max(0, r1 - r0) * std::min(SWBS, n2 - s * SWBS);
+    }
+    return c;
+}
+
+static bool band_close(const std::string& s1, const std::string& s2, int wb) {
+    constexpr int KM = 12, WIN = 32, NS = 256;
+    const int n1 = (int)s1.size(), n2 = (int)s2.size();
+    if (n1 < 4 * KM || n2 < 4 * KM) return false;
+    auto code = [](const std::string& x, int at) {
+        uint32_t v = 0;
+        for (int k = 0; k < KM; k++) v = (v << 2) | ((x[at + k] >> 1) & 3);
+        return v;
+    };
+    std::vector<uint32_t> c2(n2 - KM + 1);
+    {
+        uint32_t v = 0;
+        for (int k = 0; k < n2; k++) {
+            v = ((v << 2) | ((s2[k] >> 1) & 3)) & ((1u << (2 * KM)) - 1);
+            if (k >= KM - 1) c2[k - KM + 1] = v;
+        }
+    }
+    const int step = std::max(1, (n1 - KM) / NS);
+    int hits = 0, tries = 0, d = 0, dmax = 0;
+    for (int p = 0; p + KM <= n1; p += step) {
+        tries++;
+        const uint32_t v = code(s1, p);
+        int best = -1;
+        for (int o = 0; o <= WIN && best < 0; o++)
+            for (int sg = 0; sg < 2 && best < 0; sg++) {
+                const int q = p + d + (sg ? -o : o);
+                if (q >= 0 && q + KM <= n2 && c2[q] == v) best = q;
+            }
+        if (best >= 0) { hits++; d = best - p; dmax = std::max(dmax, std::abs(d)); }
+    }
+    return hits * 10 >= tries * 6 && 2 * dmax <= wb;
+}
+
+int sw_band_choice(const std::string& s1, const std::string& s2) {
+    const char* e = getenv("PORESEQ_SW_BAND");
+    const int mode = !e || !strcmp(e, "auto") ? 1 : (!strcmp(e, "force") ? 2 : 0);
+    const int n1 = (int)s1.size(), n2 = (int)s2.size();
+    if (!mode || n1 <= 0 || n2 <= 0 || std::min(n1, n2) > SW_PK_MAXLEN) return 0;
+    if (const char* k = getenv("PORESEQ_SW_PK")) if (atoi(k) == 0) return 0;
+    const int wb = band_width_env();
+    if (mode == 2) return wb;
+    if (2 * std::abs(n1 - n2) > wb || band_cells(n1, n2, wb) > 0.5 * (double)n1 * n2) return 0;
+    return band_close(s1, s2, wb) ? wb : 0;
+}
+
+double sw_pair_bytes(int n1, int n2, int wb) {
+    const double out = 8.0 * ((double)n1 + n2 + 2);
+    if (!wb) return 4.0 * (((double)n1 / 64 + 1) * (n2 + 8) + ((double)n2 / 64 + 1) * (n1 + 1)) + out;
+    const double nbb = SWBS / 64 + 2 * wb / 64, ns = (n2 + SWBS - 1) / SWBS;
+    return 4.0 * (ns * nbb * (SWBS + 1) + ((double)n2 / 64 + 1) * (64 * nbb + 1)) + out;
+}
+
+static std::atomic<int64_t> g_band[5];
+
+void sw_band_counters(int64_t out[5]) { for (int k = 0; k < 5; k++) out[k] = g_band[k].load(); }
+
+int sw_launch(Runtime* rt, const std::vector<std::pair<const std::string*, const std::string*>>& in, SwJob* job, const int* wbs) {
     const int np = (int)in.size();
     job->np = np;
     if (!np) return PS_OK;
     std::vector<SwPair>& pairs = job->pairs;
     std::string& pool = job->pool;
     pairs.assign(np, SwPair());
+    std::vector<int> wb(np);
+    for (int k = 0; k < np; k++) wb[k] = wbs ? wbs[k] : sw_band_choice(*in[k].first, *in[k].second);
     int maxn2 = 1;
-    for (int k = 0; k < np; k++) maxn2 = std::max(maxn2, (int)in[k].second->size());
+    for (int k = 0; k < np; k++) if (!wb[k]) maxn2 = std::max(maxn2, (int)in[k].second->size());
     int K = live_runtimes() > 1 ? 8 : 4, WW = SWW;
     if (const char* e = getenv("PORESEQ_SW_K")) K = atoi(e) == 16 ? 16 : (atoi(e) == 8 ? 8 : 4);
     {
@@ -475,30 +620,52 @@
     }
     const int sswidth = WW * 64 * K;
     const int nss = (maxn2 + sswidth - 1) / sswidth;
+    std::vector<int> order;
+    for (int pass = 0; pass < 2; pass++)
+        for (int k = 0; k < np; k++) if ((wb[k] != 0) == (pass == 1)) order.push_back(k);
+    const int nf = np - (int)std::count_if(wb.begin(), wb.end(), [](int w) { return w != 0; }), nb = np - nf;
     int64_t row_tot = 0, col_tot = 0, blk_tot = 0, out_tot = 0;
+    job->nband = nb; job->cells = 0; job->band_cells = 0;
     for (int k = 0; k < np; k++) {
         SwPair& p = pairs[k];
         p.n1 = (int)in[k].first->size(); p.n2 = (int)in[k].second->size();
+        p.wb = wb[k];
         p.nrb = std::max(1, (p.n1 + 63) / 64);
-        p.ngw = WW * std::max(1, (p.n2 + sswidth - 1) / sswidth);
-        p.pitch = ((p.n2 + 3) / 4) * 4 + 4;
         p.s1_off = (int64_t)pool.size(); pool += *in[k].first;
         p.s2_off = (int64_t)pool.size(); pool += *in[k].second;
-        p.row_off = row_tot; row_tot += (int64_t)p.nrb * p.pitch;
-        p.col_off = col_tot; col_tot += ((int64_t)p.n2 / 64 + 1) * (p.n1 + 1);
-        p.blk_off = blk_tot; blk_tot += (int64_t)p.nrb * p.ngw;
+        if (!p.wb) {
+            p.ngw = WW * std::max(1, (p.n2 + sswidth - 1) / sswidth);
+            p.pitch = ((p.n2 + 3) / 4) * 4 + 4;
+            p.nbb = p.nrb;
+            p.cpitch = p.n1 + 1;
+            p.row_off = row_tot; row_tot += (int64_t)p.nrb * p.pitch;
+            p.blk_off = blk_tot; blk_tot += (int64_t)p.nrb * p.ngw;
+            job->band_cells += (double)p.n1 * p.n2;
+        } else {
+            p.ngw = std::max(1, (p.n2 + SWBS - 1) / SWBS);
+            p.pitch = SWBS;
+            p.nbb = SWBS / 64 + 2 * p.wb / 64;
+            p.cpitch = 64 * p.nbb + 1;
+            p.row_off = row_tot; row_tot += (int64_t)p.ngw * p.nbb * SWBS;
+            p.blk_off = blk_tot; blk_tot += (int64_t)p.ngw * p.nbb;
+            job->band_cells += band_cells(p.n1, p.n2, p.wb);
+        }
+        p.col_off = col_tot; col_tot += ((int64_t)p.n2 / 64 + 1) * p.cpitch;
         p.out_off = out_tot; out_tot += 2 * ((int64_t)p.n1 + p.n2 + 2);
         p.res_off = (int64_t)k * 8;
         job->cells += (double)p.n1 * p.n2;
     }
     pool.push_back(0);
     job->out_tot = out_tot;
+    std::vector<SwPair> dev(np);
+    for (int k = 0; k < np; k++) dev[k] = pairs[order[k]];
+    const size_t nprog = (size_t)nf * (nss + 1) + 1;
     PS_TRY(rt->buf("sw_pairs").ensure(np * sizeof(SwPair)));
     PS_TRY(rt->buf("sw_chars").ensure(pool.size()));
     PS_TRY(rt->buf("sw_row").ensure(row_tot * sizeof(int)));
     PS_TRY(rt->buf("sw_col").ensure(col_tot * sizeof(int)));
     PS_TRY(rt->buf("sw_blk").ensure(blk_tot * sizeof(int)));
-    PS_TRY(rt->buf("sw_prog").ensure((size_t)np * (nss + 1) * sizeof(int)));
+    PS_TRY(rt->buf("sw_prog").ensure(nprog * sizeof(int)));
     PS_TRY(rt->buf("sw_out").ensure(out_tot * sizeof(int)));
     PS_TRY(rt->buf("sw_res").ensure((size_t)np * 8 * sizeof(int)));
     SwPair* d_pairs = rt->buf("sw_pairs").as<SwPair>();
@@ -507,36 +674,45 @@
     int* d_col = rt->buf("sw_col").as<int>();
     int* d_blk = rt->buf("sw_blk").as<int>();
     int* d_prog = rt->buf("sw_prog").as<int>();
-    int* d_ticket = d_prog + (size_t)np * nss;
+    int* d_ticket = d_prog + (size_t)nf * nss;
     int* d_out = rt->buf("sw_out").as<int>();
     int* d_res = rt->buf("sw_res").as<int>();
     hipStream_t st = nullptr;
     PS_TRY(second_stream(rt, &st));
     job->stream = st;
-    PS_TRY(rt->up(d_pairs, pairs.data(), np * sizeof(SwPair), st));
+    PS_TRY(rt->up(d_pairs, dev.data(), np * sizeof(SwPair), st));
     PS_TRY(rt->up(d_chars, pool.data(), pool.size(), st));
     PS_HIP(hipMemsetAsync(d_res, 0, (size_t)np * 8 * sizeof(int), st));
     PS_HIP(hipMemsetAsync(d_blk, 0, blk_tot * sizeof(int), st));
-    PS_HIP(hipMemsetAsync(d_prog, 0, (size_t)np * (nss + 1) * sizeof(int), st));
+    PS_HIP(hipMemsetAsync(d_prog, 0, nprog * sizeof(int), st));
     if (rt->prof_on) PS_HIP(hipEventRecord(rt->sw0, st));
-    bool packed = K == 8 && WW == SWW;
-    for (int k = 0; k < np && packed; k++) if (std::min(pairs[k].n1, pairs[k].n2) > SW_PK_MAXLEN) packed = false;
-    if (const char* e = getenv("PORESEQ_SW_PK")) if (atoi(e) == 0) packed = false;
-    if (packed) {
-        PS_TRY(sw_run_pk(rt, st, np, nss, d_pairs, d_chars, d_row, d_col, d_blk, d_prog, d_ticket, d_out, d_res));
-        if (rt->prof_on) rt->prof["sw_pk8"].launches++;
-    } else if (WW == SWW1) {
-        switch (K) {
-            case 8: PS_TRY((sw_run<8, SWW1>(rt, st, np, nss, d_pairs, d_chars, d_row, d_col, d_blk, d_prog, d_ticket, d_out, d_res))); break;
-            default: PS_TRY((sw_run<16, SWW1>(rt, st, np, nss, d_pairs, d_chars, d_row, d_col, d_blk, d_prog, d_ticket, d_out, d_res))); break;
-        }
-    } else {
-        switch (K) {
-            case 4: PS_TRY((sw_run<4, SWW>(rt, st, np, nss, d_pairs, d_chars, d_row, d_col, d_blk, d_prog, d_ticket, d_out, d_res))); break;
-            case 16: PS_TRY((sw_run<16, SWW>(rt, st, np, nss, d_pairs, d_chars, d_row, d_col, d_blk, d_prog, d_ticket, d_out, d_res))); break;
-            default: PS_TRY((sw_run<8, SWW>(rt, st, np, nss, d_pairs, d_chars, d_row, d_col, d_blk, d_prog, d_ticket, d_out, d_res))); break;
-        }
-    }
+    bool packed_all = true;
+    if (nf) {
+        bool packed = K == 8 && WW == SWW;
+        for (int k = 0; k < nf && packed; k++) if (std::min(dev[k].n1, dev[k].n2) > SW_PK_MAXLEN) packed = false;
+        if (const char* e = getenv("PORESEQ_SW_PK")) if (atoi(e) == 0) packed = false;
+        if (packed) {
+            PS_TRY(sw_run_pk(rt, st, nf, nss, d_pairs, d_chars, d_row, d_col, d_blk, d_prog, d_ticket, d_out, d_res));
+        } else if (WW == SWW1) {
+            packed_all = false;
+            switch (K) {
+                case 8: PS_TRY((sw_run<8, SWW1>(rt, st, nf, nss, d_pairs, d_chars, d_row, d_col, d_blk, d_prog, d_ticket, d_out, d_res))); break;
+                default: PS_TRY((sw_run<16, SWW1>(rt, st, nf, nss, d_pairs, d_chars, d_row, d_col, d_blk, d_prog, d_ticket, d_out, d_res))); break;
+            }
+        } else {
+            packed_all = false;
+            switch (K) {
+                case 4: PS_TRY((sw_run<4, SWW>(rt, st, nf, nss, d_pairs, d_chars, d_row, d_col, d_blk, d_prog, d_ticket, d_out, d_res))); break;
+                case 16: PS_TRY((sw_run<16, SWW>(rt, st, nf, nss, d_pairs, d_chars, d_row, d_col, d_blk, d_prog, d_ticket, d_out, d_res))); break;
+                default: PS_TRY((sw_run<8, SWW>(rt, st, nf, nss, d_pairs, d_chars, d_row, d_col, d_blk, d_prog, d_ticket, d_out, d_res))); break;
+            }
+        }
+    }
+    if (nb) {
+        PS_TRY(sw_run_band(rt, st, nb, d_pairs + nf, d_chars, d_row, d_col, d_blk, d_out, d_res));
+        if (rt->prof_on) rt->prof["sw_band"].launches++;
+    }
+    if (rt->prof_on && packed_all) rt->prof["sw_pk8"].launches++;
     if (rt->prof_on) PS_HIP(hipEventRecord(rt->sw1, st));
     PS_TRY(rt->hbuf("sw_res").ensure((size_t)np * 8 * sizeof(int)));
     PS_TRY(rt->hbuf("sw_out").ensure((size_t)out_tot * sizeof(int)));
@@ -561,6 +737,14 @@
     }
     for (int k = 0; k < np; k++)
         if (job->res[k * 8 + 5]) return fail(PS_ERR_HIP, "Smith-Waterman: a strip gave up waiting for its left neighbour (result discarded)");
+    std::vector<int> redo;
+    int edge = 0;
+    for (int k = 0; k < np; k++) {
+        const SwPair& p = job->pairs[k];
+        if (!p.wb) continue;
+        if (job->res[k * 8 + 6]) { redo.push_back(k); continue; }
+        if (job->res[k * 8 + 0] > 0 && std::abs(job->res[k * 8 + 1] - job->res[k * 8 + 2]) > p.wb - 64) edge++;
+    }
     for (int k = 0; k < np; k++) {
         const int n = job->res[k * 8 + 3], nm = job->res[k * 8 + 4];
         const SwPair& p = job->pairs[k];
@@ -572,12 +756,31 @@
         std::reverse(r.a.begin(), r.a.end()); std::reverse(r.b.begin(), r.b.end());
         r.accuracy = 100.0 * nm / (double)n;
     }
+    g_band[0] += job->nband; g_band[1] += (int64_t)redo.size(); g_band[2] += edge;
+    g_band[3] += (int64_t)job->band_cells; g_band[4] += (int64_t)job->cells;
+    static const bool trace = getenv("PORESEQ_TRACE") != nullptr;
+    if (trace && job->nband)
+        fprintf(stderr, "[ps] smith-waterman band: %d of %d pairs banded, %zu fell back, %d maxima near a band edge, %.3g of %.3g cells\n",
+                job->nband, np, redo.size(), edge, job->band_cells, job->cells);
+    if (redo.empty()) return PS_OK;
+    std::vector<std::string> s(2 * redo.size());
+    SwInput in2;
+    for (size_t k = 0; k < redo.size(); k++) {
+        const SwPair& p = job->pairs[redo[k]];
+        s[2 * k].assign(job->pool, (size_t)p.s1_off, (size_t)p.n1);
+        s[2 * k + 1].assign(job->pool, (size_t)p.s2_off, (size_t)p.n2);
+    }
+    for (size_t k = 0; k < redo.size(); k++) in2.push_back({&s[2 * k], &s[2 * k + 1]});
+    const std::vector<int> full(redo.size(), 0);
+    std::vector<SwResult> part;
+    PS_TRY(sw_batch(rt, in2, &part, full.data()));
+    for (size_t k = 0; k < redo.size(); k++) (*out)[redo[k]] = std::move(part[k]);
     return PS_OK;
 }
 
-int sw_batch(Runtime* rt, const std::vector<std::pair<const std::string*, const std::string*>>& in, std::vector<SwResult>* out) {
+int sw_batch(Runtime* rt, const std::vector<std::pair<const std::string*, const std::string*>>& in, std::vector<SwResult>* out, const int* wb) {
     SwJob job;
-    PS_TRY(sw_launch(rt, in, &job));
+    PS_TRY(sw_launch(rt, in, &job, wb));
     return sw_finish(rt, &job, out);
 }
 
```
